# eitan3/xna-ray-trace

Hardware: AMD Instinct MI355X
Metric: Mrays/sec (primary+shadow), 1920×1080; 1/2/4/8-GPU scaling vs HBM roofline (higher is better)
Workload: dtype f32

## Files before the change

### include/xrt.h

```cpp
#ifndef XRT_H
#define XRT_H

#include <stdint.h>

#ifdef __cplusplus
extern "C" {
#endif

#define XRT_VERSION 203

#define XRT_OK              0
#define XRT_E_INVALID_ARG  -1
#define XRT_E_BUSY         -2
#define XRT_E_NO_DEVICE    -3
#define XRT_E_OOM          -4
#define XRT_E_HIP          -5
#define XRT_E_RCCL         -6
#define XRT_E_INTERNAL     -7
#define XRT_E_UNSUPPORTED  -8
#define XRT_E_NOT_BUILT    -9

#define XRT_FILTER_POINT     0
#define XRT_FILTER_BILINEAR  1
#define XRT_ADDRESS_CLAMP    0
// ... 139 lines not shown
                               void *stream);

int xrt_mesh_intersect(xrt_scene *scene, int32_t mesh_id, const xrt_ray *rays, int64_t n,
                       xrt_hit *hits_out);

int xrt_render(xrt_scene *scene, const xrt_camera *camera, const xrt_light *lights, int32_t n_lights,
               const xrt_render_opts *opts, uint32_t *rgba_out, float *rgb_f32_out,
               xrt_stats *stats_out );

int xrt_render_begin(xrt_scene *scene, const xrt_camera *camera, const xrt_light *lights, int32_t n_lights,
                     const xrt_render_opts *opts, uint32_t *rgba_out, int32_t *ticket_out);
int xrt_render_end(xrt_scene *scene, int32_t ticket, xrt_stats *stats_out);

int xrt_host_register(void *host_ptr, uint64_t bytes);
int xrt_host_unregister(void *host_ptr);

int xrt_render_device(xrt_scene *scene, const xrt_camera *camera, const xrt_light *lights,
                      int32_t n_lights, const xrt_render_opts *opts, void *d_rgba_out,
                      void *stream, xrt_stats *stats_out );

int xrt_render_device_begin(xrt_scene *scene, const xrt_camera *camera, const xrt_light *lights,
                            int32_t n_lights, const xrt_render_opts *opts, void *d_rgba_out, void *stream,
                            int32_t *ticket_out);
int xrt_render_device_end(xrt_scene *scene, int32_t ticket, xrt_stats *stats_out);

#define XRT_TILE_W 64
#define XRT_TILE_H 8
int xrt_shard_layout(int32_t width, int32_t height, int32_t shard_count, int32_t *tiles_x_out,
                     int32_t *tiles_y_out, int32_t *tiles_per_rank_out);


int xrt_scene_set_tile_table(xrt_scene *scene, int32_t width, int32_t height, int32_t shard_count, int32_t tiles_per_rank,
                             const int32_t *tile_of_slot);

int xrt_scene_tile_costs(xrt_scene *scene, int32_t width, int32_t height, float *cost_out, int32_t reset);

int xrt_balance_tiles(int32_t width, int32_t height, int32_t shard_count, const float *tile_cost, int32_t tiles_per_rank,
                      int32_t *tile_of_slot_out);

int xrt_detile_table_device(int32_t width, int32_t height, int32_t shard_count, int32_t tiles_per_rank, const void *d_tile_of_slot,
                            const void *d_gathered, int64_t rank_stride, void *d_rgba_out, void *stream);

int xrt_detile_device(int32_t width, int32_t height, int32_t shard_count, const void *d_gathered, int64_t rank_stride,
                      void *d_rgba_out, void *stream);

int xrt_rccl_probe(void);

int xrt_split_stats(xrt_scene *scene, uint64_t out[4], int32_t reset);

int xrt_debug_end_counts(xrt_scene *scene, uint64_t out[3]);

int xrt_debug_packet_table(xrt_scene *scene, uint64_t counts[2], uint32_t *entries_out, int64_t entries_cap, int32_t *paths_out, int64_t paths_cap);

float xrt_progress(const xrt_scene *scene);

int xrt_generate_primary_rays(xrt_scene *scene, const xrt_camera *camera, xrt_ray *rays_out );

int xrt_cast_rays(xrt_scene *scene, const xrt_ray *rays, int64_t n, int32_t iteration, float current_ref_index,
                  const xrt_light *lights, int32_t n_lights, const xrt_render_opts *opts,
                  uint32_t *rgba_out, float *rgb_f32_out, xrt_stats *stats_out );

int xrt_cast_rays_device(xrt_scene *scene, const void *d_rays, int64_t n, int32_t iteration, float current_ref_index,
                         const xrt_light *lights, int32_t n_lights, const xrt_render_opts *opts,
                         void *d_rgba_out, void *d_rgb_f32_out, void *stream, xrt_stats *stats_out );

int xrt_shade_hits(xrt_scene *scene, const xrt_ray *rays, const xrt_hit *hits, int64_t n,
                   int32_t iteration, float current_ref_index,
                   const xrt_light *lights, int32_t n_lights, const xrt_render_opts *opts,
                   uint32_t *rgba_out, float *rgb_f32_out , xrt_stats *stats_out );

int xrt_shade_hits_device(xrt_scene *scene, const void *d_rays, const void *d_hits, int64_t n,
                          int32_t iteration, float current_ref_index,
                          const xrt_light *lights, int32_t n_lights, const xrt_render_opts *opts,
                          void *d_rgba_out, void *d_rgb_f32_out , void *stream,
                          xrt_stats *stats_out );

int xrt_light_hits(xrt_scene *scene, const xrt_hit *hits, int64_t n,
                   const xrt_light *lights, int32_t n_lights,
                   float *light_f32_out , float *amount_out ,
                   xrt_stats *stats_out );

int xrt_light_hits_device(xrt_scene *scene, const void *d_hits, int64_t n,
                          const xrt_light *lights, int32_t n_lights,
                          void *d_light_f32_out, void *d_amount_out , void *stream,
                          xrt_stats *stats_out );

#define XRT_SURF_HIT          1
#define XRT_SURF_TRANSPARENT  2
#define XRT_SURF_INTERPOLATED 4
#define XRT_SURF_TEXTURED     8

typedef struct xrt_surface {
    float   normal[3];
    float   reflectiveness;
    float   color[3];
    float   alpha;
    float   uv[2];
    float   refraction_index;
    float   next_ref_index;
    int32_t flags;
    int32_t reserved[3];
} xrt_surface;

int xrt_surface_hits(xrt_scene *scene, const xrt_ray *rays , const xrt_hit *hits, int64_t n,
                     float current_ref_index, const xrt_render_opts *opts,
                     xrt_surface *surface_out , xrt_ray *reflect_out ,
// ... 85 lines not shown
```

### xna-ray-trace_amd/_abi.py

```python
import ctypes as C
import os

_HERE = os.path.dirname(os.path.abspath(__file__))
import re


def _lib_name():
    v = os.environ.get("XRT_LIB_VARIANT", "libxrt.so")
    if not re.fullmatch(r"libxrt(_\w+)?\.so", v):
        raise ImportError("XRT_LIB_VARIANT=%r: expected libxrt[_name].so (a file inside %s)" % (v, os.path.join(_HERE, "csrc")))
    return v


LIB_PATH = os.path.join(_HERE, "csrc", _lib_name())

XRT_OK = 0
XRT_E_INVALID_ARG = -1
XRT_E_BUSY = -2
XRT_E_NO_DEVICE = -3
XRT_E_OOM = -4
XRT_E_HIP = -5
XRT_E_RCCL = -6
XRT_E_INTERNAL = -7
XRT_E_UNSUPPORTED = -8
# ... 64 lines not shown
    _fields_ = [("position", C.c_float * 3), ("color", C.c_uint32)]


class xrt_surface(C.Structure):
    _fields_ = [("normal", C.c_float * 3), ("reflectiveness", C.c_float), ("color", C.c_float * 3), ("alpha", C.c_float),
                ("uv", C.c_float * 2), ("refraction_index", C.c_float), ("next_ref_index", C.c_float), ("flags", C.c_int32),
                ("reserved", C.c_int32 * 3)]


SURF_HIT, SURF_TRANSPARENT, SURF_INTERPOLATED, SURF_TEXTURED = 1, 2, 4, 8
SURFACE_DTYPE = [("normal", "<f4", 3), ("reflectiveness", "<f4"), ("color", "<f4", 3), ("alpha", "<f4"), ("uv", "<f4", 2),
                 ("refraction_index", "<f4"), ("next_ref_index", "<f4"), ("flags", "<i4"), ("reserved", "<i4", 3)]
assert C.sizeof(xrt_surface) == 64
assert C.sizeof(xrt_path_vertex) == 16
assert C.sizeof(xrt_ray) == 32 and C.sizeof(xrt_hit) == 48 and C.sizeof(xrt_render_opts) == 48
XRT_VERSION = 203

_P = C.POINTER
_F = _P(C.c_float)
SYMBOLS = {
    "xrt_version": (C.c_int, []),
    "xrt_last_error": (C.c_char_p, []),
    "xrt_device_count": (C.c_int, [_P(C.c_int)]),
    "xrt_scene_create": (C.c_int, [C.c_int, _P(C.c_void_p)]),
    "xrt_scene_destroy": (C.c_int, [C.c_void_p]),
    "xrt_scene_add_mesh": (C.c_int, [C.c_void_p, _F, _F, _F, _F, _F, C.c_int32, _P(xrt_material), _F, _P(C.c_int32)]),
    "xrt_scene_add_object": (C.c_int, [C.c_void_p, _P(C.c_int32), C.c_int32, _F, _F, _F, _F, _P(C.c_int32)]),
    "xrt_scene_build": (C.c_int, [C.c_void_p, C.c_int32, C.c_int32]),
    "xrt_scene_save": (C.c_int, [C.c_void_p, C.c_char_p]),
    "xrt_scene_load": (C.c_int, [C.c_int, C.c_char_p, _P(C.c_void_p)]),
    "xrt_scene_get_tree": (C.c_int, [C.c_void_p, C.c_int32, _P(xrt_node_info), _P(C.c_int64), _P(C.c_int32), _P(C.c_int64)]),
    "xrt_scene_intersect": (C.c_int, [C.c_void_p, _P(xrt_ray), _P(C.c_int32), C.c_int64, _P(xrt_hit), _P(xrt_stats)]),
    "xrt_scene_intersect_device": (C.c_int, [C.c_void_p, C.c_void_p, C.c_int64, C.c_void_p, C.c_void_p]),
    "xrt_mesh_intersect": (C.c_int, [C.c_void_p, C.c_int32, _P(xrt_ray), C.c_int64, _P(xrt_hit)]),
    "xrt_render": (C.c_int, [C.c_void_p, _P(xrt_camera), _P(xrt_light), C.c_int32, _P(xrt_render_opts), _P(C.c_uint32), _F, _P(xrt_stats)]),
    "xrt_render_begin": (C.c_int, [C.c_void_p, _P(xrt_camera), _P(xrt_light), C.c_int32, _P(xrt_render_opts), _P(C.c_uint32), _P(C.c_int32)]),
    "xrt_render_end": (C.c_int, [C.c_void_p, C.c_int32, _P(xrt_stats)]),
    "xrt_host_register": (C.c_int, [C.c_void_p, C.c_uint64]),
    "xrt_host_unregister": (C.c_int, [C.c_void_p]),
    "xrt_render_device": (C.c_int, [C.c_void_p, _P(xrt_camera), _P(xrt_light), C.c_int32, _P(xrt_render_opts), C.c_void_p, C.c_void_p, _P(xrt_stats)]),
    "xrt_render_device_begin": (C.c_int, [C.c_void_p, _P(xrt_camera), _P(xrt_light), C.c_int32, _P(xrt_render_opts), C.c_void_p, C.c_void_p, _P(C.c_int32)]),
    "xrt_render_device_end": (C.c_int, [C.c_void_p, C.c_int32, _P(xrt_stats)]),
    "xrt_shard_layout": (C.c_int, [C.c_int32, C.c_int32, C.c_int32, _P(C.c_int32), _P(C.c_int32), _P(C.c_int32)]),
    "xrt_detile_device": (C.c_int, [C.c_int32, C.c_int32, C.c_int32, C.c_void_p, C.c_int64, C.c_void_p, C.c_void_p]),
    "xrt_scene_set_tile_table": (C.c_int, [C.c_void_p, C.c_int32, C.c_int32, C.c_int32, C.c_int32, _P(C.c_int32)]),
    "xrt_scene_tile_costs": (C.c_int, [C.c_void_p, C.c_int32, C.c_int32, _F, C.c_int32]),
    "xrt_balance_tiles": (C.c_int, [C.c_int32, C.c_int32, C.c_int32, _F, C.c_int32, _P(C.c_int32)]),
    "xrt_detile_table_device": (C.c_int, [C.c_int32, C.c_int32, C.c_int32, C.c_int32, C.c_void_p, C.c_void_p, C.c_int64, C.c_void_p, C.c_void_p]),
    "xrt_progress": (C.c_float, [C.c_void_p]),
    "xrt_rccl_probe": (C.c_int, []),
    "xrt_split_stats": (C.c_int, [C.c_void_p, _P(C.c_uint64), C.c_int32]),
    "xrt_debug_end_counts": (C.c_int, [C.c_void_p, _P(C.c_uint64)]),
    "xrt_debug_packet_table": (C.c_int, [C.c_void_p, _P(C.c_uint64), _P(C.c_uint32), C.c_int64, _P(C.c_int32), C.c_int64]),
    "xrt_generate_primary_rays": (C.c_int, [C.c_void_p, _P(xrt_camera), _P(xrt_ray)]),
    "xrt_cast_rays": (C.c_int, [C.c_void_p, _P(xrt_ray), C.c_int64, C.c_int32, C.c_float, _P(xrt_light), C.c_int32, _P(xrt_render_opts),
                                _P(C.c_uint32), _F, _P(xrt_stats)]),
    "xrt_cast_rays_device": (C.c_int, [C.c_void_p, C.c_void_p, C.c_int64, C.c_int32, C.c_float, _P(xrt_light), C.c_int32, _P(xrt_render_opts),
                                       C.c_void_p, C.c_void_p, C.c_void_p, _P(xrt_stats)]),
    "xrt_shade_hits": (C.c_int, [C.c_void_p, _P(xrt_ray), _P(xrt_hit), C.c_int64, C.c_int32, C.c_float, _P(xrt_light), C.c_int32,
                                 _P(xrt_render_opts), _P(C.c_uint32), _F, _P(xrt_stats)]),
    "xrt_shade_hits_device": (C.c_int, [C.c_void_p, C.c_void_p, C.c_void_p, C.c_int64, C.c_int32, C.c_float, _P(xrt_light), C.c_int32,
                                        _P(xrt_render_opts), C.c_void_p, C.c_void_p, C.c_void_p, _P(xrt_stats)]),
    "xrt_light_hits": (C.c_int, [C.c_void_p, _P(xrt_hit), C.c_int64, _P(xrt_light), C.c_int32, _F, _F, _P(xrt_stats)]),
    "xrt_light_hits_device": (C.c_int, [C.c_void_p, C.c_void_p, C.c_int64, _P(xrt_light), C.c_int32, C.c_void_p, C.c_void_p, C.c_void_p, _P(xrt_stats)]),
    "xrt_surface_hits": (C.c_int, [C.c_void_p, _P(xrt_ray), _P(xrt_hit), C.c_int64, C.c_float, _P(xrt_render_opts), _P(xrt_surface), _P(xrt_ray), _P(xrt_ray),
                                   _P(xrt_stats)]),
    "xrt_surface_hits_device": (C.c_int, [C.c_void_p, C.c_void_p, C.c_void_p, C.c_int64, C.c_float, _P(xrt_render_opts), C.c_void_p, C.c_void_p, C.c_void_p,
                                          C.c_void_p, _P(xrt_stats)]),
    "xrt_compose_hits": (C.c_int, [C.c_void_p, _P(xrt_surface), _F, _P(C.c_uint32), _P(C.c_uint32), C.c_int64, _P(C.c_uint32), _F, _P(xrt_stats)]),
    "xrt_compose_hits_device": (C.c_int, [C.c_void_p, C.c_void_p, C.c_void_p, C.c_void_p, C.c_void_p, C.c_int64, C.c_void_p, C.c_void_p, C.c_void_p,
                                          _P(xrt_stats)]),
    "xrt_fold_samples": (C.c_int, [C.c_void_p, _P(C.c_uint32), C.c_int64, C.c_int32, _P(C.c_uint32), _F, _P(xrt_stats)]),
    "xrt_fold_samples_device": (C.c_int, [C.c_void_p, C.c_void_p, C.c_int64, C.c_int32, C.c_void_p, C.c_void_p, C.c_void_p, _P(xrt_stats)]),
    "xrt_cast_rays_paths": (C.c_int, [C.c_void_p, _P(xrt_ray), C.c_int64, C.c_int32, C.c_float, _P(xrt_light), C.c_int32, _P(xrt_render_opts),
                                      _P(C.c_uint32), _F, _P(xrt_ray), _P(C.c_int64), _P(xrt_path_vertex), C.c_int64, _P(C.c_int64), _P(xrt_stats)]),
    "xrt_cast_rays_paths_device": (C.c_int, [C.c_void_p, C.c_void_p, C.c_int64, C.c_int32, C.c_float, _P(xrt_light), C.c_int32, _P(xrt_render_opts),
                                             C.c_void_p, C.c_void_p, C.c_void_p, C.c_void_p, C.c_void_p, C.c_int64, C.c_void_p, _P(C.c_int64), _P(xrt_stats)]),
    "xrt_scene_set_poses": (C.c_int, [C.c_void_p, _P(C.c_int32), C.c_int32, _F, _F, _F]),
    "xrt_scene_set_poses_device": (C.c_int, [C.c_void_p, C.c_void_p, C.c_int32, C.c_void_p, C.c_void_p, C.c_void_p, C.c_void_p]),
    "xrt_scene_build_tree": (C.c_int, [C.c_void_p, C.c_int32]),
    "xrt_scene_set_materials": (C.c_int, [C.c_void_p, _P(C.c_int32), C.c_int32, _P(xrt_material)]),
    "xrt_scene_set_bodies": (C.c_int, [C.c_void_p, C.c_int32, _P(C.c_int32), _P(C.c_int32), _P(C.c_float), _P(C.c_float), _P(C.c_float),
                                       _P(C.c_float), C.c_int32, _P(C.c_int32)]),
    "xrt_scene_set_triangle_shading": (C.c_int, [C.c_void_p, C.c_int32, _P(C.c_int32), C.c_int32, C.c_int32, _F, _F, _F]),
    "xrt_scene_set_triangle_shading_device": (C.c_int, [C.c_void_p, C.c_int32, C.c_void_p, C.c_int32, C.c_int32, C.c_void_p, C.c_void_p, C.c_void_p,
                                                        C.c_void_p]),
    "xrt_render_pixels": (C.c_int, [C.c_void_p, _P(xrt_camera), _P(xrt_light), C.c_int32, _P(xrt_render_opts), _F, C.c_int64, _P(C.c_uint32), _F,
                                    _P(xrt_stats)]),
    "xrt_render_pixels_device": (C.c_int, [C.c_void_p, _P(xrt_camera), _P(xrt_light), C.c_int32, _P(xrt_render_opts), C.c_void_p, C.c_int64,
                                           C.c_void_p, C.c_void_p, C.c_void_p, _P(xrt_stats)]),
    "xrt_trace_pixels": (C.c_int, [C.c_void_p, _P(xrt_camera), _P(xrt_render_opts), _F, C.c_int64, _P(xrt_ray), _P(xrt_hit), _P(xrt_stats)]),
    "xrt_trace_pixels_device": (C.c_int, [C.c_void_p, _P(xrt_camera), _P(xrt_render_opts), C.c_void_p, C.c_int64, C.c_void_p, C.c_void_p, C.c_void_p,
                                          _P(xrt_stats)]),
}

_lib = None


class XrtError(RuntimeError):
    def __init__(self, code, msg):
        super().__init__("libxrt error %d: %s" % (code, msg))
        self.code = code


def lib():
    global _lib
# ... 28 lines not shown
```

### xna-ray-trace_amd/api.py

```python
import ctypes as C
import threading
import numpy as np

from . import _abi as abi
from . import xna

f32 = np.float32


def _fp(a):
    return a.ctypes.data_as(C.POINTER(C.c_float))


def _material_property(name, convert, texels=False):
    attr = "_" + name

    def get(self):
        return getattr(self, attr)

    def set_(self, value):
        setattr(self, attr, convert(value))
        self._serial = getattr(self, "_serial", 0) + 1
        if texels:
            self._tex_serial = getattr(self, "_tex_serial", 0) + 1
# ... 440 lines not shown
        some = next((t for t in (ids, normals, uv, color) if t is not None), None)
        s = stream if stream is not None else torch.cuda.current_stream(some.device if some is not None else None)
        ptr = lambda t: C.c_void_p(t.data_ptr()) if t is not None else None
        abi.check(abi.lib().xrt_scene_set_triangle_shading_device(self.handle, int(mesh_id), ptr(ids), first, n, ptr(normals), ptr(uv), ptr(color),
                                                                  C.c_void_p(s.cuda_stream)))
        if 0 <= mesh_id < len(self.meshes):
            hids = np.arange(first, first + n, dtype=np.int64) if ids is None else ids.detach().cpu().numpy()
            keep = (hids >= 0) & (hids < self.meshes[mesh_id].data.ntri)
            host = lambda t, shape: None if t is None else t.detach().cpu().numpy().reshape(shape)[keep]
            self._mirror_triangle_shading(int(mesh_id), hids[keep], 0, int(keep.sum()), host(normals, (n, 3, 3)), host(uv, (n, 3, 2)),
                                          host(color, (n, 4)))

    def Save(self, path):
        self._push_materials()
        abi.check(abi.lib().xrt_scene_save(self.handle, str(path).encode()))

    @classmethod
    def Load(cls, path, device=0):
        sm = cls(device)
        sm._scene = _Scene.__new__(_Scene)
        sm._scene.handle = C.c_void_p()
        abi.check(abi.lib().xrt_scene_load(int(device), str(path).encode(), C.byref(sm._scene.handle)))
        abi.check(abi.lib().xrt_scene_build(sm._scene.handle, sm.meshItemTreshold, sm.itemTreshold))
        return sm

    @property
    def handle(self):
        if self._scene is None:
            raise RuntimeError("scene not built")
        return self._scene.handle

    def mesh_id(self, mesh):
        return self._mesh_ids[id(mesh)]

    def SplitStats(self, reset=True):
        out = (C.c_uint64 * 4)()
        abi.check(abi.lib().xrt_split_stats(self.handle, out, 1 if reset else 0))
        return tuple(int(x) for x in out)

    def EndCounts(self):
        out = (C.c_uint64 * 3)()
        abi.check(abi.lib().xrt_debug_end_counts(self.handle, out))
        return tuple(int(x) for x in out)

    def PacketTable(self):
        counts = (C.c_uint64 * 2)()
        abi.check(abi.lib().xrt_debug_packet_table(self.handle, counts, None, 0, None, 0))
        entries = np.zeros((int(counts[0]), 2), dtype=np.uint32)
        paths = np.zeros(int(counts[1]), dtype=np.int32)
        abi.check(abi.lib().xrt_debug_packet_table(self.handle, counts, entries.ctypes.data_as(C.POINTER(C.c_uint32)), entries.shape[0],
                                                   paths.ctypes.data_as(C.POINTER(C.c_int32)), paths.shape[0]))
        return entries, paths

    def IntersectBatch(self, rays, stats=False):
        rays = np.ascontiguousarray(rays, dtype=RAY_DTYPE)
        hits = np.zeros(rays.shape[0], dtype=HIT_DTYPE)
        st = abi.xrt_stats()
        self._push_poses()
        self._push_materials()
        abi.check(abi.lib().xrt_scene_intersect(self.handle, rays.ctypes.data_as(C.POINTER(abi.xrt_ray)), None, rays.shape[0],
                                                hits.ctypes.data_as(C.POINTER(abi.xrt_hit)), C.byref(st) if stats else None))
        return (hits, st.as_dict()) if stats else hits

    def GetRayIntersection(self, ray, ignoreTriangle=None, ignoreObject=None):
        im, it = (-1, -1) if ignoreTriangle is None else (self.mesh_id(ignoreTriangle[0]), int(ignoreTriangle[1]))
        h = self.IntersectBatch(rays_array([ray[0]], [ray[1]], im, it))[0]
        if not h["hit"]:
            return False, None
        return True, dict(mesh=self.meshes[h["mesh"]], triangle=int(h["tri"]), u=h["u"], v=h["v"], d=h["d"],
                          worldPosition=h["w"].copy(), object=int(h["object"]), leaf=int(h["leaf"]))

    def tree(self, mesh=None):
        return _get_tree(self._scene, -1 if mesh is None else self.mesh_id(mesh))


class Camera:

    def __init__(self, position, target, up, fieldOfView, aspectRatio, nearClippingPlane, farClippingPlane):
        self.Position, self.Target, self.Up = position, target, up
        self.FieldOfView, self.AspectRatio = fieldOfView, aspectRatio
        self.NearClippingPlane, self.FarClippingPlane = nearClippingPlane, farClippingPlane

    @property
    def View(self):
        return xna.as_array(xna.create_look_at(self.Position, self.Target, self.Up))

    @property
    def Projection(self):
        return xna.as_array(xna.create_perspective_fov(self.FieldOfView, self.AspectRatio, self.NearClippingPlane, self.FarClippingPlane))


class SpotLight:
    IsPositionable = True

    def __init__(self):
        self.Position = (0.0, 0.0, 0.0)
        self.Direction = (0.0, -1.0, 0.0)
        self.Color = (1.0, 1.0, 1.0)
        self.DecayExponent = 1.3
        self.Intensity = 1.0
        self.SpotAngle = 0.0

    def _to_abi(self):
        l = abi.xrt_light()
        l.kind = abi.LIGHT_SPOT
        l.position[:] = self.Position
# ... 520 lines not shown
```

### xna-ray-trace_amd/csrc/frame_plan.h

```cpp
#pragma once
#include "../../include/xrt.h"
#include "kernels.h"

struct xrt_scene;
namespace xrt { struct PixelGenArgs; }

struct BatchSrc {
    const xrt_ray *rays = nullptr;
    long long n = 0;
    float refIndex = 1.0f;
    struct Paths {
        xrt_path_vertex *vertices = nullptr;
        long long capacity = 0;
        long long *vertexStart = nullptr;
        xrt_ray *raysBack = nullptr;
    };
    const Paths *paths = nullptr;
    const xrt_hit *hits = nullptr;
    bool coherent = false;
    int samples = 1;
    const xrt::PixelGenArgs *gen = nullptr;
};

constexpr int ADAPTIVE_LEVEL_WORDS = 16;

struct FramePlan {
    xrt::RayGenParams g{};
    int R = 0, nL = 0;
    int addressMode = 0, filtering = 0;
    bool tabled = false;
    long long totalTiles = 0, myTiles = 0, totalPixels = 0;
    long long framePaths = 0;
    long long partStart = 0, firstPaths = 0;
    long long hintPaths = -1;
    unsigned long long validPixels = 0;
    size_t nodes = 0;
    long long chunkPaths = 0;
    int P = 0;
    size_t rayCap = 0, liveCap = 0, lvlStride = 0, shadowCap = 0;
    int cntStride = 0, qStride = 0;
    bool lvlVerified = false;
    bool heap = false;
    bool adaptive = false;
    int quality = 0;
    bool batch = false, capturePaths = false;
    bool givenHits = false;
    bool collect = false;
    bool fast = false;
    bool heapFast = false;
    bool adaptiveFast = false;
    bool ae = false;
    bool finishA = false;
    bool endEarly = false;
    bool skipTiles = false;
    unsigned long long endSkipped = 0;
    bool fuseResolve = false;
    bool wantF32 = false;
    bool wantFeedback = false;
    bool listLong = false;
    bool hinted = false;
    bool tileCosts = false;
    bool useStamps = false;
    int pkMask = 0;
    size_t pkEntries = 0;
    int shadeBlock = 1024;
    bool ownStream = false;
    int cntBase = 0, levelCap = 0;
};

int plan_frame(const xrt_scene &s, int matVersion, const xrt_camera *cam, const xrt_light *lights, int nLights, const xrt_render_opts *opts, bool wantsF32,
               bool hasStream, int part, int nParts, bool heapFastAllowed, const BatchSrc *batch, FramePlan &plan);

int scene_packet_mask(const xrt_scene &s, int samples);
bool scene_answers_at_emission(const xrt_scene &s);
```

### xna-ray-trace_amd/csrc/kernels.h

```cpp
#pragma once
#include <hip/hip_runtime.h>

#include "../../include/xrt.h"
#include "traverse.h"

namespace xrt {

struct ShadeView {
    const f4 *shade;
    const MaterialRec *materials;
    const uint32_t *texels;
    const MeshRec *meshes;
    const LightRec *lights;
    int nLights;
    int addressMode, filtering;
};

struct HeavyArgs {
    int *list = nullptr;
    int *count = nullptr;
    float path = 0.0f;
    const unsigned *costMap = nullptr;
    unsigned epoch = 0;
    int costThreshold = 0;
// ... 17 lines not shown
    int batchMax = 64;
    int heavyShift = 3;
    int batchMin = 64;
    int spreadMin = 4;
    unsigned long long *stamps = nullptr;
    const xrt_ray *rays2 = nullptr;
    xrt_hit *hits2 = nullptr;
    const int *nDev2 = nullptr;
    int nMul2 = 0, nCap2 = 0;
    int *flags = nullptr, *flags2 = nullptr;
    int missRecords = 0;
    const int *scatter = nullptr, *scatter2 = nullptr;
};

constexpr int STAMP_HEADER = 2, STAMP_SLOTS = 8192, STAMP_STRIDE = STAMP_HEADER + STAMP_SLOTS;

struct alignas(16) SlotRec { float wx, wy, wz; int path; float nx, ny, nz, refl; };
struct PacketArgs {
    const xrt_ray *rays = nullptr;
    xrt_hit *hits = nullptr;
    const int *index = nullptr;
    const int *nDev = nullptr;
    int nMul = 1, n = 0, nCap = 0;
    unsigned *queue = nullptr;
    int mode = MODE_SINGLE, meshId = 0;
    int unmark = 0;
    int staticDiv = 4;
    int grabMax = 2;
    int *flags = nullptr;
    int splitLong = 0, splitBudgetLong = 0;
    int cullMin = 4;
    unsigned long long *stamps = nullptr;
    const xrt_ray *rays2 = nullptr;
    xrt_hit *hits2 = nullptr;
    int *flags2 = nullptr;
    const int *nDev2 = nullptr;
    int nMul2 = 0, nCap2 = 0;
    const int *scatter = nullptr, *scatter2 = nullptr;
    unsigned *tileCost = nullptr;
    int tileShift = 9, nL1 = 1, nL2 = 1, tileBase = 0;
    const int *pathOf1 = nullptr;
    const SlotRec *slotOf1 = nullptr;
    const SlotRec *slotOf2 = nullptr;
    unsigned *splitCtl = nullptr;
    unsigned *splitItems = nullptr;
    unsigned *splitRecs = nullptr;
    int splitNI = 0, splitNR = 0;
    unsigned splitSerial = 0;
    int splitBudget = 0, splitBudgetItem = 0;
    unsigned *splitCost = nullptr;
    const uint2 *pkTable = nullptr;
    const unsigned *pkCount = nullptr;
    int pkCap = 0;
};
struct QuadTable {
    uint2 *table = nullptr;
    unsigned *count = nullptr, *clear = nullptr;
    int cap = 0;
};
constexpr int QUAD_HEAD_WORDS = 128;
constexpr int PACKET_QUEUE_HEADS = 8, PACKET_HEAD_STRIDE = 64;
constexpr int PACKET_SPLIT_WORDS = 320;
constexpr int PACKET_QUEUE_WORDS = PACKET_QUEUE_HEADS * PACKET_HEAD_STRIDE + PACKET_SPLIT_WORDS;
constexpr int SPLIT_HEAD_WORDS = 32, SPLIT_PART_WORDS = 7 * 64, SPLIT_ITEM_WORDS = SPLIT_HEAD_WORDS + 64 + SPLIT_PART_WORDS, SPLIT_REC_HEAD = 64, SPLIT_REC_WORDS = SPLIT_REC_HEAD + SPLIT_PART_WORDS;
constexpr int SPLIT_REC_ITEMS = 32;
int  packet_split_stats(unsigned long long out[4], bool reset);
bool packet_supported(int mode, int meshDepth, int sceneDepth);
int  packet_blocks_per_cu(int mode);
void launch_packet(const SceneView &S, const PacketArgs &A, int gridBlocks, hipStream_t st, hipEvent_t e0 = nullptr, hipEvent_t e1 = nullptr);

enum { C_RAYS = 0, C_HITS, C_SCENE_NODES, C_INSTANCES, C_MESH_AABB, C_MESH_QUERIES, C_NODES, C_REFS, C_TRIS, C_MESH_AWAY, C_COUNT };

constexpr int FLAG_MISS = 0, FLAG_HIT = 1, FLAG_TRANSPARENT = 2;


enum { END_LISTED = 0, END_BY_RAYGEN, END_BY_SHADE, END_WORDS };
struct EndArgs {
    int on = 0;
    uint32_t *sampleColor = nullptr;
    int *list = nullptr, *cnt = nullptr;
    int listCap = 0;
    int skipTiles = 0;
};

struct ShadeArgs {
    int level, doA, doB;
    int maxReflections, P, heap;
    int *overflow;
    const xrt_ray *rays; const xrt_hit *hits;
    const int *nDev; int nHost, cap;
    const int *index, *rayPath, *rayNode; const float *rayRef;
    SlotRec *slotOut; int *slotNodeOut; int *scnt; int shadowCap; xrt_ray *shadowRays;
    xrt_ray *nextRays; int *nextPath, *nextNode; float *nextRef; int *nextCnt; int nextCap;
    const SlotRec *slotPrev; const int *slotNodePrev; const int *scntPrev; const xrt_hit *shadowHits;
    f4 *lvlA, *lvlB; float *lvlAlpha;
    LvlMap lvl;
    HeavyArgs heavy;
    unsigned *costOut = nullptr;
    unsigned epoch = 0;
    const int *hitFlags = nullptr, *shadowFlags = nullptr;
    int ae = 0;
    int *shadowCnt = nullptr, *shadowOut = nullptr, *shadowFlagsOut = nullptr;
    int finish = 0;
    int *finishCnt = nullptr;
    EndArgs end;
};

void launch_intersect(const SceneView &S, const IntersectArgs &A, int stackNeeded, int gridBlocks, hipStream_t st, hipEvent_t e0 = nullptr,
                      hipEvent_t e1 = nullptr);
int  intersect_blocks_per_cu(int stackNeeded, int mode);
void launch_count(const SceneView &S, const IntersectArgs &A, unsigned long long *counters, hipStream_t st);
void launch_raygen(const RayGenParams &g, const SceneView &S, xrt_ray *rays, f4 *lvlB0, int *index, int *count, int P, long long pathBase,
// ... 93 lines not shown
```

### xna-ray-trace_amd/csrc/kernels.hip

```cpp
#include "kernels.h"
#include "device_util.h"
#include "pose.h"
#include "shade_math.h"

#include <hip/hip_ext.h>

namespace xrt {

struct LdsStack {
    unsigned *base;
    __device__ __forceinline__ unsigned get(int i) const { return base[i * 64]; }
    __device__ __forceinline__ void set(int i, unsigned v) { base[i * 64] = v; }
};

__device__ __forceinline__ int wave_scan_max(int v) {
    v = max(v, __builtin_amdgcn_update_dpp(0, v, 0x111, 0xf, 0xf, false));
    v = max(v, __builtin_amdgcn_update_dpp(0, v, 0x112, 0xf, 0xf, false));
    v = max(v, __builtin_amdgcn_update_dpp(0, v, 0x114, 0xf, 0xf, false));
    v = max(v, __builtin_amdgcn_update_dpp(0, v, 0x118, 0xf, 0xf, false));
    v = max(v, __builtin_amdgcn_update_dpp(0, v, 0x142, 0xa, 0xf, false));
    v = max(v, __builtin_amdgcn_update_dpp(0, v, 0x143, 0xc, 0xf, false));
    return v;
}

constexpr int APPEND_BLOCK = 1024;
__device__ __forceinline__ int block_append(int *counter, bool flag, int *ldsCounts ) {
    const unsigned long long m = __ballot(flag);
    const int wave = (int)(threadIdx.x >> 6), nw = (int)(blockDim.x >> 6), lane = lane_id();
    if (lane == 0) ldsCounts[wave] = (int)__popcll(m);
    __syncthreads();
    if (wave == 0) {
        const int c = lane < nw ? ldsCounts[lane] : 0;
        const int incl = wave_scan_add(c);
        const int total = __builtin_amdgcn_readlane(incl, 63);
        int base = 0;
        if (lane == 0 && total) base = atomicAdd(counter, total);
        base = __builtin_amdgcn_readfirstlane(base);
        if (lane < nw) ldsCounts[lane] = base + incl - c;
    }
    __syncthreads();
    const int slot = ldsCounts[wave] + lanes_below(m);
    __syncthreads();
    return slot;
}

__device__ __forceinline__ void block_count(int *counter, int n, int *ldsCounts ) {
    const int wave = (int)(threadIdx.x >> 6), nw = (int)(blockDim.x >> 6), lane = lane_id();
    const int mine = __builtin_amdgcn_readlane(wave_scan_add(n), 63);
    __syncthreads();
    if (lane == 0) ldsCounts[wave] = mine;
    __syncthreads();
    if (wave == 0) {
        const int total = __builtin_amdgcn_readlane(wave_scan_add(lane < nw ? ldsCounts[lane] : 0), 63);
        if (lane == 0 && total) atomicAdd(counter, total);
    }
// ... 483 lines not shown
            const int q = grp * span + r * APPEND_BLOCK + (int)threadIdx.x;
            const int p = path_of(q);
            bool live = false, heavy = false, record = true;
            keepO[r] = mk(0, 0, 0); keepD[r] = mk(0, 0, 0);
            if (q < walk && p < P) {
                long long gp = pathBase + p;
                const int sshift = g.samples == 16 ? 4 : (g.samples == 4 ? 2 : 0);
                int s = (int)(gp & (long long)(g.samples - 1));
                int x = 0, y = 0;
                const bool listed = g.quadLevel > 0;
                if (!listed && !path_pixel(g, gp >> sshift, x, y)) {
                    if (!index) store_ray(rays + p, mk(0, 0, 0), mk(0, 0, 0), DEAD_RAY, -1);
                    record = g.cullSkipsRecord == 0;
                } else if (index && !listed && (x < g.cullX0 || x > g.cullX1 || y < g.cullY0 || y > g.cullY1)) {
                    record = g.cullSkipsRecord == 0;
                } else {
                    float sx = (float)x, sy = (float)y;
                    if (g.quadLevel >= 0) {
                        if (listed) { sx = g.quadCx[gp >> 2]; sy = g.quadCy[gp >> 2]; }
                        const float quarter = g.quadSize * 0.25f;
                        sx = (s & 1) ? sx + quarter : sx - quarter;
                        sy = (s & 2) ? sy + quarter : sy - quarter;
                    } else if (g.samples == 16) {
                        int q = s >> 2, rr = s & 3;
                        sx = (sx + ((q & 1) ? 0.25f : -0.25f)) + ((rr & 1) ? 0.125f : -0.125f);
                        sy = (sy + ((q & 2) ? 0.25f : -0.25f)) + ((rr & 2) ? 0.125f : -0.125f);
                    }
                    v3 nearP = unproject(g, sx, sy, 0.0f);
                    v3 farP = unproject(g, sx, sy, 1.0f);
                    v3 dir = normalize(sub(farP, nearP));
                    if (index) {
                        RayPre w = make_ray(nearP, dir);
                        float key;
                        live = slab(w, rlo.x, rlo.y, rlo.z, rhi.x, rhi.y, rhi.z, key);
                    }
                    heavy = live && H.list && long_ray(S, H, p, nearP, dir);
                    if (!index) store_ray(rays + p, nearP, dir, -1, -1);
                    keepO[r] = nearP; keepD[r] = dir;
                }
                if constexpr (END) { if (!live) { sample_color_out(E.sampleColor, nullptr, p, pack_color(mk(0, 0, 0)), mk(0, 0, 0)); nEnded++; } }
                else if (index && !live && record) lvlB0[lvl_at(g.lvl, p)] = f4{0, 0, 0, i2f(FLAG_MISS)};
            }
            const unsigned long long ml = __ballot(live), mh = __ballot(heavy);
            liveAt[r] = live ? lanes_below(ml) : -1;
            heavyAt[r] = heavy ? lanes_below(mh) : -1;
            if (lane == 0) { ldsLive[r * 16 + wave] = (int)__popcll(ml); ldsHeavy[r * 16 + wave] = (int)__popcll(mh); }
        }
        if (!index) continue;
        __syncthreads();
        int quadLen = 0, quadAt = 0;
        if (wave == 0 && Q.table) reserve_cells_and_entries(ldsLive, count, Q.count, quadLen, quadAt);
        else if (wave < 2 && (wave == 0 || H.list)) reserve_cells(wave == 0 ? ldsLive : ldsHeavy, wave == 0 ? count : H.count);
        __syncthreads();
        if (quadLen > 0 && quadAt < Q.cap) Q.table[quadAt] = make_uint2((unsigned)ldsLive[lane], (unsigned)quadLen);
#pragma unroll
        for (int r = 0; r < RG_ROUNDS; r++) {
            const int p = path_of(grp * span + r * APPEND_BLOCK + (int)threadIdx.x);
            if (liveAt[r] >= 0) {
                const int slot = ldsLive[r * 16 + wave] + liveAt[r];
                if (slot < liveCap) {
                    index[slot] = p;
                    store_ray(rays + slot, keepO[r], keepD[r], -1, heavyAt[r] >= 0 ? (-1 ^ HEAVY_BIT) : -1);
                    if (heavyAt[r] >= 0) H.list[ldsHeavy[r * 16 + wave] + heavyAt[r]] = slot;
                }
            }
        }
        __syncthreads();
    }
    if constexpr (END) block_count(E.cnt + END_BY_RAYGEN, nEnded, ldsLive);
}
__global__ __launch_bounds__(APPEND_BLOCK) void k_ingest(RayGenParams g, SceneView S, xrt_ray *rays, f4 *lvlB0, int *index, int *count, int P,
                                                         long long pathBase, HeavyArgs H, int liveCap) {
    __shared__ int ldsLive[RG_ROUNDS * 16], ldsHeavy[RG_ROUNDS * 16];
    const f4 rlo = S.snodes[0], rhi = S.snodes[1];
    const int span = RG_ROUNDS * APPEND_BLOCK;
    const int groups = (P + span - 1) / span;
    const int wave = (int)(threadIdx.x >> 6), lane = lane_id();
    for (int grp = (int)blockIdx.x; grp < groups; grp += (int)gridDim.x) {
        int liveAt[RG_ROUNDS], heavyAt[RG_ROUNDS];
        f4 keepA[RG_ROUNDS], keepB[RG_ROUNDS];
#pragma unroll
        for (int r = 0; r < RG_ROUNDS; r++) {
            const int p = grp * span + r * APPEND_BLOCK + (int)threadIdx.x;
            bool live = false, heavy = false;
            keepA[r] = f4{0, 0, 0, 0}; keepB[r] = f4{0, 0, 0, 0};
            if (p < P) {
                const f4 *src = g.batch + 2 * (size_t)(pathBase + p);
                const f4 a = src[0], b = src[1];
                const v3 o = mk(a.x, a.y, a.z), d = mk(a.w, b.x, b.y);
                int im = f2i(b.z), it = f2i(b.w);
                if (it < 0 || im < 0 || im >= S.nMeshes || it >= S.meshes[im].ntri) { im = -1; it = -1; }
                RayPre w = make_ray(o, d);
                float key;
                live = slab(w, rlo.x, rlo.y, rlo.z, rhi.x, rhi.y, rhi.z, key);
                heavy = live && H.list && long_ray(S, H, p, o, d);
                keepA[r] = a;
                keepB[r] = f4{b.x, b.y, i2f(im), i2f(heavy ? (it ^ HEAVY_BIT) : it)};
                if (!live) lvlB0[p] = f4{0, 0, 0, i2f(FLAG_MISS)};
            }
            const unsigned long long ml = __ballot(live), mh = __ballot(heavy);
            liveAt[r] = live ? lanes_below(ml) : -1;
            heavyAt[r] = heavy ? lanes_below(mh) : -1;
            if (lane == 0) { ldsLive[r * 16 + wave] = (int)__popcll(ml); ldsHeavy[r * 16 + wave] = (int)__popcll(mh); }
        }
        __syncthreads();
        if (wave < 2 && (wave == 0 || H.list)) reserve_cells(wave == 0 ? ldsLive : ldsHeavy, wave == 0 ? count : H.count);
        __syncthreads();
// ... 679 lines not shown
```

### xna-ray-trace_amd/csrc/packet.hip

```cpp
#include "device_util.h"
#include "kernels.h"

#include <hip/hip_ext.h>

namespace xrt {

constexpr int PK_LEVELS = 24;
constexpr int PK_FRAME_WORDS = 4;
constexpr int PK_SPLIT_AT = PK_LEVELS * (PK_FRAME_WORDS + 16);
constexpr int PK_STACK_WORDS = PK_SPLIT_AT + 8 + 24;
static_assert(PK_STACK_WORDS == 512, "a wave's stack is 2 KB");
constexpr int PK_SLEVELS = 12;
constexpr int PK_SFRAME_WORDS = 4;
constexpr int PK_QUEUES = 8;
static_assert(PK_QUEUES >= 1 && PK_QUEUES <= PACKET_QUEUE_HEADS, "the host zeroes PACKET_QUEUE_WORDS heads per packet launch");
#ifndef PK_SINGLE_WAVES
#define PK_SINGLE_WAVES 6
#endif
constexpr int PK_SGPRS = PK_SINGLE_WAVES >= 7 ? 96 : 112;

#if defined(XRT_PK_COUNTERS) && !defined(XRT_PK_TICKS)
#define XRT_PK_TICKS
#endif
#ifdef XRT_PK_TICKS
__device__ unsigned long long g_pkWorst[16];
__device__ unsigned g_pkDump[2 * 65536];
__device__ unsigned long long g_pkTicks[32];
#endif
#ifdef XRT_PK_COUNTERS
__device__ unsigned long long g_pkCounters[16];
__device__ unsigned g_pkCur[8 * 65536];
#define PKC(i) (pkc[i]++)
#else
#define PKC(i) ((void)0)
#endif

__device__ unsigned long long g_splitStats[4];
struct alignas(4) TriWords { float w[16]; };
__device__ __forceinline__ int rfl(int v) { return __builtin_amdgcn_readfirstlane(v); }
__device__ __forceinline__ unsigned ld_ag(const unsigned *p) { return __hip_atomic_load(p, __ATOMIC_RELAXED, __HIP_MEMORY_SCOPE_AGENT); }
__device__ __forceinline__ void st_ag(unsigned *p, unsigned v) { __hip_atomic_store(p, v, __ATOMIC_RELAXED, __HIP_MEMORY_SCOPE_AGENT); }
__device__ __forceinline__ void stores_done() { __builtin_amdgcn_fence(__ATOMIC_RELEASE, "workgroup"); asm volatile("s_waitcnt vmcnt(0)" ::: "memory"); }
__device__ __forceinline__ void loads_after() { __builtin_amdgcn_fence(__ATOMIC_ACQUIRE, "workgroup"); }
__device__ __forceinline__ unsigned xcc_id() { return (unsigned)__builtin_amdgcn_s_getreg(20 | (0 << 6) | ((4 - 1) << 11)) & 7u; }
__device__ __forceinline__ float rflf(float v) { return i2f(__builtin_amdgcn_readfirstlane(f2i(v))); }

struct PkUniform {
    int blk, p, dm0;
    unsigned long long lanes;
};
struct alignas(16) PkBlockWords { float w[PBLOCK_WORDS]; };
struct alignas(16) Frame4 { unsigned a, b, c, d; };
__device__ __forceinline__ int pk_hit8_fast(const RayPre &r, const PkBlockWords &B) {
    const float tx0 = (B.w[8] - r.o.x) * r.inv.x, tx1 = (B.w[9] - r.o.x) * r.inv.x, tx2 = (B.w[10] - r.o.x) * r.inv.x;
// ... 72 lines not shown
    L.mfound = 1;
    L.mKey = better ? L.leafKey : L.mKey; L.mDist = better ? t : L.mDist; L.mU = better ? u : L.mU; L.mV = better ? v : L.mV;
    L.mRef = better ? r : L.mRef; L.mLeaf = better ? L.leafNode : L.mLeaf;
}

template <class KeyFn>
__device__ __forceinline__ void pk_scan_leaf(const float *__restrict__ refT, int r0, int r1, Lane &L, const SceneView &S, bool keyed, KeyFn entry_key) {
    const char *pt = reinterpret_cast<const char *>(refT) + (size_t)r0 * TRI_REC_BYTES;
    auto test = [&](const TriWords &q, int r) {
        float u, v, t;
        PkTriMid m;
        if (pk_tri_pre(q, L, m)) {
            if (pk_tri_hit(q, L, m, u, v, t)) {
                if (!keyed) L.leafKey = entry_key();
                pk_candidate(L, S, r, u, v, t);
            }
        }
    };
    TriWords qA = *reinterpret_cast<const TriWords *>(pt);
    int r = r0;
    for (;;) {
        const TriWords qB = *reinterpret_cast<const TriWords *>(pt + TRI_REC_BYTES);
        test(qA, r);
        if (r + 1 >= r1) break;
        qA = *reinterpret_cast<const TriWords *>(pt + 2 * TRI_REC_BYTES);
        test(qB, r + 1);
        r += 2; pt += 2 * TRI_REC_BYTES;
        if (r >= r1) break;
    }
}

constexpr unsigned PK_KERNARG_SCENE = 8 * 8, PK_KERNARG_ARGS = PK_KERNARG_SCENE + (unsigned)sizeof(SceneView);
static_assert(sizeof(SceneView) % 8 == 0 && alignof(PacketArgs) == 8, "kernel-argument offsets of k_packet");
typedef const __attribute__((address_space(4))) PacketArgs *PkArgsK;
typedef const __attribute__((address_space(4))) SceneView *PkSceneK;
struct PkKernarg {
    unsigned long long base;
    __device__ __forceinline__ PkKernarg() : base((unsigned long long)__builtin_amdgcn_kernarg_segment_ptr()) {}
    __device__ __forceinline__ void fresh() {
        unsigned lo = (unsigned)__builtin_amdgcn_readfirstlane((int)(unsigned)base), hi = (unsigned)__builtin_amdgcn_readfirstlane((int)(unsigned)(base >> 32));
        asm volatile("" : "+s"(lo), "+s"(hi));
        base = (unsigned long long)lo | ((unsigned long long)hi << 32);
    }
    __device__ __forceinline__ PkArgsK args() const { return (PkArgsK)(base + PK_KERNARG_ARGS); }
    __device__ __forceinline__ PkSceneK scene() const { return (PkSceneK)(base + PK_KERNARG_SCENE); }
    __device__ __forceinline__ SceneView result_view() const {
        const PkSceneK k = scene();
        SceneView v = {};
        v.refG = k->refG; v.refN = k->refN; v.meshes = k->meshes; v.childDfs = k->childDfs; v.objects = k->objects;
        return v;
    }
};

template <bool SPLIT, bool LEAF_RHO>
__device__ __forceinline__ void pk_walk(const float *__restrict__ pblocks, const float *__restrict__ refT, const float *__restrict__ lrec,
                                        const SceneView &S, int cullMin, unsigned *stk, int lane, Lane &L,
                                        const RayCull &RC, bool fastL, int rootBlock, unsigned long long lanes0, bool nodeCull,
                                        bool resume) {
#ifdef XRT_PK_COUNTERS
    unsigned pkc[16] = {0, 0, 0, 0, 0, 0, 0, 0, 0, 0, 0, 0, 0, 0, 0, 0};
    pkc[0] = 1;
    pkc[12] = (unsigned)__popcll(lanes0);
#endif
    PkUniform U;
    U.blk = rootBlock;
    U.lanes = lanes0;
    U.p = 0; U.dm0 = 0;
    unsigned char *const cbOf = reinterpret_cast<unsigned char *>(stk + PK_LEVELS * PK_FRAME_WORDS) + lane;
    int sp = resume ? 1 : 0;
    bool entering = !resume, anyFound = resume && __any(L.mfound != 0);
    PkBlockWords B;
    int cb = 0;
    unsigned *const sst = stk + PK_SPLIT_AT;
    auto spill = [&]() {
        PkKernarg K;
        K.fresh();
        const PkArgsK a = K.args();
        unsigned *const ctl = a->splitCtl, *const itemsB = a->splitItems, *const recsB = a->splitRecs;
        const int NR = a->splitNR;
        const unsigned serial = a->splitSerial, xcc = xcc_id(), NIx = (unsigned)a->splitNI / 8u;
        const unsigned takerBudget = (unsigned)a->splitBudgetItem, takerEvery = (unsigned)rfl((int)sst[7]);
        int rec = rfl((int)sst[0]);
        for (int lvl = 0; lvl < sp; lvl++) {
            const Frame4 f = *reinterpret_cast<const Frame4 *>(stk + lvl * PK_FRAME_WORDS);
            const unsigned p = (unsigned)rfl((int)f.b);
            if (p == 0u) continue;
            if (rec < 0) {
                unsigned r = 0u;
                if (lane == 0) r = atomicAdd(ctl + 256, 1u);
                rec = rfl((int)r);
                if (rec >= NR) { rec = -1; break; }
                if (lane == 0) {
                    unsigned *const R0 = recsB + (size_t)rec * SPLIT_REC_WORDS;
                    (void)atomicExch(R0, 1u); (void)atomicExch(R0 + 1, 0u);
                    sst[0] = (unsigned)rec;
                    atomicAdd(&g_splitStats[2], 1ull);
                }
            }
            unsigned *const R = recsB + (size_t)rec * SPLIT_REC_WORDS;
            unsigned j = 0u, idx = 0u;
            if (lane == 0) j = atomicAdd(R + 1, 1u);
            j = (unsigned)rfl((int)j);
            if (j >= (unsigned)SPLIT_REC_ITEMS) break;
            if (lane == 0) idx = atomicAdd(ctl + 32u * xcc, 1u);
            idx = (unsigned)rfl((int)idx);
            if (idx >= NIx) { if (lane == 0) st_ag(R + 32 + j, 0xffffffffu); break; }
            idx += xcc * NIx;
// ... 35 lines not shown
                    }
                }
            }
            B = *reinterpret_cast<const PkBlockWords *>(pblocks + (size_t)U.blk * PBLOCK_WORDS);
            cb = 0;
            if (in) cb = fastL ? pk_hit8_fast(L.r, B) : pk_hit8_slow(L.r, B);
            cb &= 0xff & ~((f2i(B.w[2]) >> 8) & 0xff);
            U.dm0 = __builtin_amdgcn_readlane(L.dmask, (int)__builtin_ctzll(U.lanes));
            const int a4 = U.dm0 & 4, a2 = U.dm0 & 2, a1 = U.dm0 & 1;
            int q = cb;
            q = ((q << a4) | (q >> a4)) & 0xff;
            q = ((q & 0x33) << a2) | ((q & 0xcc) >> a2);
            q = ((q & 0x55) << a1) | ((q & 0xaa) >> a1);
            U.p = wave_or(q);
            entering = false;
        }
        if (U.p == 0) {
            if (sp == 0) break;
            sp--;
            PKC(10);
            const Frame4 f = *reinterpret_cast<const Frame4 *>(stk + sp * PK_FRAME_WORDS);
            U.blk = rfl((int)f.a); U.p = rfl((int)f.b);
            U.lanes = (unsigned long long)(unsigned)rfl((int)f.c) | ((unsigned long long)(unsigned)rfl((int)f.d) << 32);
            U.dm0 = __builtin_amdgcn_readlane(L.dmask, (int)__builtin_ctzll(U.lanes));
            B = *reinterpret_cast<const PkBlockWords *>(pblocks + (size_t)U.blk * PBLOCK_WORDS);
            cb = (int)cbOf[sp * 64];
            continue;
        }
        const int c = (int)__builtin_ctz((unsigned)U.p) ^ U.dm0;
        U.p &= U.p - 1;
        PKC(2);
        const bool inC = in && ((cb >> c) & 1);
        const int d0 = f2i(B.w[0]), d1 = f2i(B.w[1]), d2 = f2i(B.w[2]), d3 = f2i(B.w[3]);
        auto entry_key = [&]() {
            v3 cmin, cmax;
            pk_child_box(B, c, cmin, cmax);
            float k = 0.0f;
            if (fastL) (void)slab_fast(L.r, L.dmask, cmin, cmax, k);
            else (void)slab(L.r, cmin.x, cmin.y, cmin.z, cmax.x, cmax.y, cmax.z, k);
            return k;
        };
        const bool keyed = anyFound;
        float key = 0.0f;
        if (keyed && inC) key = entry_key();
#ifdef XRT_PK_COUNTERS
        if (keyed) pkc[11]++;
        pkc[13] += (unsigned)__popcll(__ballot(inC));
#endif
        const int node = U.blk * 8 + c;
        if (!((d2 >> c) & 1)) {
            PKC(3);
            const f4 *const nr = reinterpret_cast<const f4 *>(lrec + (size_t)node * LREC_WORDS);
            const f4 nlo = nr[0], nhi = nr[1];
            bool go = inC & !all_back_facing(nlo, nhi, L.r.d);
            if (keyed) go = go & !((L.mfound != 0) & (key > L.mKey));
            if (!__any(go)) continue;
            PKC(4);
            const unsigned long long offLo = (unsigned long long)(unsigned)f2i(B.w[4]) | ((unsigned long long)(unsigned)f2i(B.w[5]) << 32);
            const unsigned long long offHi = (unsigned long long)(unsigned)f2i(B.w[6]) | ((unsigned long long)(unsigned)f2i(B.w[7]) << 32);
            const int r0 = d1 + child_ref_offset(offLo, offHi, c);
            const int r1 = d1 + ((c == 7) ? d3 : child_ref_offset(offLo, offHi, c + 1));
            const bool big = r1 - r0 >= LEAF_RUN_MIN;
            float rho = 0.0f;
            bool usable = false;
            if constexpr (LEAF_RHO) {
                if (big || r1 - r0 >= cullMin) {
                    usable = leaf_margin(L.r, RC, nr[2], nr[3], nr[4], nr[5], rho);
                    if (r1 - r0 >= cullMin) {
                        go = go && !(usable && grown_box_missed(L.r, nr[2], nr[3], rho));
                        if (!__any(go)) continue;
                    }
                }
            } else if (r1 - r0 >= cullMin) {
                go = go && !leaf_certainly_missed_fused(L.r, RC, nr[2], nr[3], nr[4], nr[5]);
                if (!__any(go)) continue;
            }
            PKC(5);
            int nRuns = 1, rb = -1;
            if (big) { rb = f2i(lrec[(size_t)node * LREC_WORDS + 24]); if (rb >= 0) nRuns = (r1 - r0 + LEAF_RUN - 1) / LEAF_RUN; }
            const bool cheap = LEAF_RHO && !__any(go && !usable);
            for (int jr = 0; jr < nRuns; jr++) {
                int ra = r0, rz = r1;
                bool goR = go;
                if (rb >= 0) {
                    ra = r0 + LEAF_RUN * jr; rz = min(ra + LEAF_RUN, r1);
                    const f4 *tb = reinterpret_cast<const f4 *>(lrec + (size_t)rb + (size_t)jr * RUN_WORDS);
                    PKC(6);
                    if (cheap) goR = go && !grown_box_missed(L.r, tb[0], tb[1], rho);
                    else if constexpr (LEAF_RHO) goR = go && !leaf_certainly_missed(L.r, RC, tb[0], tb[1], tb[2], tb[3]);
                    else goR = go && !leaf_certainly_missed_fused(L.r, RC, tb[0], tb[1], tb[2], tb[3]);
                    if (!__any(goR)) continue;
                }
                PKC(7);
#ifdef XRT_PK_COUNTERS
                pkc[8] += (unsigned)(rz - ra);
                pkc[14] += (unsigned)(rz - ra) * (unsigned)__popcll(__ballot(goR));
#endif
                if (goR) {
                    L.leafKey = key; L.leafNode = node;
                    const char *pt = reinterpret_cast<const char *>(refT) + (size_t)ra * TRI_REC_BYTES;
                    auto test = [&](const TriWords &q, int r) {
                        float u, v, t;
                        PkTriMid m;
                        if (pk_tri_pre(q, L, m)) {
                            if (pk_tri_hit(q, L, m, u, v, t)) {
                                if (!keyed) L.leafKey = entry_key();
                                pk_candidate(L, S, r, u, v, t);
                            }
                        }
                    };
                    TriWords qA = *reinterpret_cast<const TriWords *>(pt);
                    int r = ra;
                    for (;;) {
                        const TriWords qB = *reinterpret_cast<const TriWords *>(pt + TRI_REC_BYTES);
                        test(qA, r);
                        if (r + 1 >= rz) break;
                        qA = *reinterpret_cast<const TriWords *>(pt + 2 * TRI_REC_BYTES);
                        test(qB, r + 1);
                        r += 2; pt += 2 * TRI_REC_BYTES;
                        if (r >= rz) break;
                    }
                }
            }
            if (!keyed) anyFound = __any(L.mfound != 0);
            continue;
        }
        bool go = inC;
        if (keyed && ((d2 >> (16 + c)) & 1)) go = go & !((L.mfound != 0) & (key > L.mKey));
        if (nodeCull && ((d2 >> (24 + c)) & 1)) {
            const f4 *const nr = reinterpret_cast<const f4 *>(lrec + (size_t)node * LREC_WORDS);
            go = go && !all_back_facing(nr[0], nr[1], L.r.d);
            PKC(9);
        }
        const unsigned long long LL = __ballot(go);
        if (LL == 0ull) continue;
        if (sp >= PK_LEVELS - 1) continue;
        if (U.p != 0) {
            cbOf[sp * 64] = (unsigned char)cb;
            if (lane == 0) *reinterpret_cast<Frame4 *>(stk + sp * PK_FRAME_WORDS) = Frame4{(unsigned)U.blk, (unsigned)U.p, (unsigned)U.lanes, (unsigned)(U.lanes >> 32)};
            __builtin_amdgcn_fence(__ATOMIC_RELEASE, "wavefront");
            __builtin_amdgcn_wave_barrier();
            __builtin_amdgcn_fence(__ATOMIC_ACQUIRE, "wavefront");
            sp++;
        }
        U.blk = d0 + __builtin_popcount((unsigned)(d2 & 0xff) & ((1u << c) - 1u));
        U.lanes = LL;
        entering = true;
    }
#ifdef XRT_PK_COUNTERS
    if (lane == 0) for (int i = 0; i < 16; i++) if (pkc[i]) atomicAdd(&g_pkCounters[i], (unsigned long long)pkc[i]);
    if (lane == 0) {
        unsigned *cur = g_pkCur + 8 * ((blockIdx.x * 4 + (threadIdx.x >> 6)) & 65535);
        cur[0] += pkc[0]; cur[1] += pkc[1]; cur[2] += pkc[2]; cur[3] += pkc[8]; cur[4] += pkc[6];
    }
#endif
}

constexpr int PK_PARK_WORDS = 19;
struct PkScene {
    LdsRay w;
    LdsField<float> sKey;
    LdsField<int> sfound;
    LdsField<float> sbKey, sbD, sbU, sbV;
    LdsField<int> sbRef, sbLeaf, sbObj, sbMesh;
    int obj;
    __device__ __forceinline__ explicit PkScene(unsigned *b)
        : w{b}, sKey{b + 9 * 64}, sfound{b + 10 * 64}, sbKey{b + 11 * 64}, sbD{b + 12 * 64}, sbU{b + 13 * 64}, sbV{b + 14 * 64},
          sbRef{b + 15 * 64}, sbLeaf{b + 16 * 64}, sbObj{b + 17 * 64}, sbMesh{b + 18 * 64}, obj(-1) {}
};
template <int M> __device__ __forceinline__ unsigned *scene_park() {
    if constexpr (M == MODE_SCENE) { __shared__ unsigned mem[4 * PK_PARK_WORDS * 64]; return mem; }
    else return nullptr;
}
template <int M> __device__ __forceinline__ unsigned *scene_frames() {
    if constexpr (M == MODE_SCENE) { __shared__ unsigned mem[4 * PK_SLEVELS * PK_SFRAME_WORDS]; return mem; }
    else return nullptr;
}

#ifndef PK_SCENE_WAVES
#define PK_SCENE_WAVES 5
#endif
template <int M, bool SP>
__global__ __launch_bounds__(256, (M == MODE_SCENE) ? PK_SCENE_WAVES : (PK_SINGLE_WAVES >= 7 ? 7 : (SP ? 6 : 1))) __attribute__((amdgpu_num_sgpr(PK_SGPRS))) void k_packet(const float *__restrict__ pblocks, const float *__restrict__ refT,
                                                const float *__restrict__ lrec, const MeshRec *__restrict__ meshes,
                                                const f4 *__restrict__ snodes, const f4 *__restrict__ scull, const ObjRec *__restrict__ objects,
                                                const int *__restrict__ objMesh, SceneView S, PacketArgs A) {
    __shared__ unsigned frames[4 * PK_STACK_WORDS];
    unsigned *const sframesAll = scene_frames<M>();
    unsigned *const parkAll = scene_park<M>();
    stamp_begin(A.stamps);
    PkKernarg KA;
    const int lane = lane_id(), wave = (int)(threadIdx.x >> 6);
    unsigned *const stk = &frames[wave * PK_STACK_WORDS];
    int n = A.nDev ? (*A.nDev) * A.nMul : A.n;
    if (A.nCap > 0 && n > A.nCap) n = A.nCap;
    int n2 = A.nDev2 ? (*A.nDev2) * A.nMul2 : 0;
    if (n2 > A.nCap2) n2 = A.nCap2;
    int nPkT = (n + 63) >> 6;
    if (A.pkTable) { const int t = (int)*A.pkCount; nPkT = t > A.pkCap ? A.pkCap : t; }
    const int nPk1 = nPkT, nPk = nPk1 + ((n2 + 63) >> 6);
    const int nWaves = (int)gridDim.x * 4, waveId = (int)blockIdx.x * 4 + wave;
    int staticPer = A.staticDiv > 0 ? nPk / (nWaves * A.staticDiv) : 0;
    if (staticPer == 0) staticPer = 1;
    const int qBase = min(nWaves * staticPer, nPk);
    const int dynTotal = nPk - qBase;
    unsigned dead = 0u;
    for (int h = 0; h < PK_QUEUES; h++) if (dynTotal - h <= 0) dead |= 1u << h;
    int cur = waveId % PK_QUEUES, seen = 0, curR = cur;
    int sNext = 0, dNext = 0, dEnd = 0;
    constexpr bool splitOn = SP && M != MODE_SCENE;
    unsigned *const sst = stk + PK_SPLIT_AT;
    if (splitOn && lane == 0) sst[2] = 0u;
    bool mainDone = false;
    for (;;) {
        int pk = -1, item = -1;
        bool contended = false;
        if (splitOn) {
            KA.fresh();
            const unsigned xcc = xcc_id(), NIx = (unsigned)KA.args()->splitNI / 8u;
            unsigned *const ctl = KA.args()->splitCtl + 32u * xcc;
            unsigned long long th = 0ull;
            if (lane == 0) th = __hip_atomic_load(reinterpret_cast<unsigned long long *>(ctl), __ATOMIC_RELAXED, __HIP_MEMORY_SCOPE_AGENT);
            const unsigned t = (unsigned)rfl((int)(unsigned)th), h = (unsigned)rfl((int)(unsigned)(th >> 32));
            if (h < (t < NIx ? t : NIx)) {
                unsigned old = 0u;
                if (lane == 0) old = atomicCAS(ctl + 1, h, h + 1u);
                if ((unsigned)rfl((int)old) == h) item = (int)(xcc * NIx + h);
                else contended = true;
            }
        }
        if (item < 0) {
            if (mainDone) {
                if (!contended) break;
                __builtin_amdgcn_s_sleep(8);
                continue;
            }
// ... 65 lines not shown
#else
        const bool costed = KA.args()->tileCost != nullptr || (splitOn && KA.args()->splitCost != nullptr);
#endif
        const unsigned long long tPacket = costed ? wall_clock64() : 0ull;
        const bool seg2 = pk >= nPk1;
        int w = (seg2 ? pk - nPk1 : pk) * 64 + lane;
        bool valid = w < (seg2 ? n2 : n);
        if (!seg2) {
            const uint2 *const tab = KA.args()->pkTable;
            if (tab) {
                const uint2 e = tab[pk];
                w = rfl((int)e.x) + lane;
                valid = lane < rfl((int)e.y) && w < n;
            }
        }
        const xrt_ray *const raysS = seg2 ? KA.args()->rays2 : KA.args()->rays;
        Lane L;
        L.state = ST_FINISH; L.mfound = 0; L.cost = 0; L.rayIndex = 0; L.mesh = 0; L.weird = 0; L.dmask = 0; L.ignoreId = -1; L.mask = 0;
        L.r = make_ray(mk(0, 0, 0), mk(1, 1, 1));
        int idx = 0;
        v3 o = mk(0, 0, 0), d = mk(0, 0, 0);
        int im = DEAD_RAY, it = -1;
        if (valid) {
            const int *const indexL = KA.args()->index;
            idx = (indexL && !seg2) ? indexL[w] : w;
            load_ray(raysS + idx, o, d, im, it);
            if (KA.args()->unmark && heavy_marked(it)) it ^= HEAVY_BIT;
        }
        if constexpr (M != MODE_SCENE) {
            SceneLane C;
            C.sfound = 0; C.obj = 0;
            if (valid && im != DEAD_RAY) lane_begin(L, C, S, o, d, im, it, idx, M, A.meshId, false);
            const RayCull RC = make_ray_cull(L.r.o, L.r.d);
            const int mesh = (M == MODE_MESH) ? A.meshId : 0;
            const MeshRec &mr = meshes[mesh];
            const bool fastL = L.r.par == 0 && L.weird == 0;
            const bool nodeCull = S.nodeCull == 2 || (S.nodeCull == 1 && __any(valid && L.ignoreId >= 0));
            const bool meshAway = nodeCull && mesh_faces_away(mr, L.r.d);
            unsigned long long lanes0 = mr.rootBlock < 0 ? 0ull : __ballot(valid && L.state == ST_NODE && L.mask != 0 && !meshAway);
            if (splitOn) {
                if (item >= 0) {
                    const unsigned *const P = itemW + SPLIT_HEAD_WORDS + 64 + lane;
                    L.mfound = (int)ld_ag(P); L.mKey = i2f((int)ld_ag(P + 64)); L.mDist = i2f((int)ld_ag(P + 128)); L.mU = i2f((int)ld_ag(P + 192)); L.mV = i2f((int)ld_ag(P + 256));
                    L.mRef = (int)ld_ag(P + 320); L.mLeaf = (int)ld_ag(P + 384);
                    reinterpret_cast<unsigned char *>(stk + PK_LEVELS * PK_FRAME_WORDS)[lane] = (unsigned char)ld_ag(itemW + SPLIT_HEAD_WORDS + lane);
                    const unsigned hw = lane < 4 ? ld_ag(itemW + 3 + lane) : 0u;
                    if (lane < 4) stk[lane] = hw;
                    lanes0 = (unsigned long long)(unsigned)__builtin_amdgcn_readlane((int)hw, 2) | ((unsigned long long)(unsigned)__builtin_amdgcn_readlane((int)hw, 3) << 32);
                    __builtin_amdgcn_fence(__ATOMIC_RELEASE, "wavefront");
                    __builtin_amdgcn_wave_barrier();
                    __builtin_amdgcn_fence(__ATOMIC_ACQUIRE, "wavefront");
                }
            }
            pk_walk<splitOn, true>(pblocks, refT, lrec, S, A.cullMin, stk, lane, L, RC, fastL, mr.rootBlock, lanes0, nodeCull, splitOn && item >= 0);
            L.mesh = mesh;
            KA.fresh();
            bool mine = true;
            if (splitOn) {
                const int rec = rfl((int)sst[0]);
                if (rec >= 0) {
                    const int itemA = rfl((int)sst[1]);
                    unsigned *const R = KA.args()->splitRecs + (size_t)rec * SPLIT_REC_WORDS;
                    unsigned *const P = (itemA >= 0 ? KA.args()->splitItems + (size_t)itemA * SPLIT_ITEM_WORDS + SPLIT_HEAD_WORDS + 64 : R + SPLIT_REC_HEAD) + lane;
                    st_ag(P, (unsigned)L.mfound); st_ag(P + 64, (unsigned)f2i(L.mKey)); st_ag(P + 128, (unsigned)f2i(L.mDist)); st_ag(P + 192, (unsigned)f2i(L.mU)); st_ag(P + 256, (unsigned)f2i(L.mV));
                    st_ag(P + 320, (unsigned)L.mRef); st_ag(P + 384, (unsigned)L.mLeaf);
                    stores_done();
                    unsigned left = 0u;
                    if (lane == 0) left = atomicSub(R, 1u);
                    mine = rfl((int)left) == 1;
                    if (mine) {
                        loads_after();
                        if (itemA >= 0 && lane == 0) atomicAdd(&g_splitStats[3], 1ull);
                        const SceneView Sr = KA.result_view();
                        int nIt = rfl((int)__hip_atomic_load(R + 1, __ATOMIC_RELAXED, __HIP_MEMORY_SCOPE_AGENT));
                        if (nIt > SPLIT_REC_ITEMS) nIt = SPLIT_REC_ITEMS;
                        for (int j = -1; j < nIt; j++) {
                            const unsigned *Q = R + SPLIT_REC_HEAD + lane;
                            if (j >= 0) {
                                const unsigned ix = (unsigned)rfl((int)ld_ag(R + 32 + j));
                                if (ix == 0xffffffffu) continue;
                                Q = KA.args()->splitItems + (size_t)ix * SPLIT_ITEM_WORDS + SPLIT_HEAD_WORDS + 64 + lane;
                            }
                            const int qf = (int)ld_ag(Q), qRef = (int)ld_ag(Q + 320), qLeaf = (int)ld_ag(Q + 384);
                            const float qKey = i2f((int)ld_ag(Q + 64)), qD = i2f((int)ld_ag(Q + 128)), qU = i2f((int)ld_ag(Q + 192)), qV = i2f((int)ld_ag(Q + 256));
                            if (qf != 0) {
                                bool better = (L.mfound == 0) | (qKey < L.mKey) | ((qKey == L.mKey) & (qD < L.mDist));
                                if ((L.mfound != 0) & (qKey == L.mKey) & (qD == L.mDist))
                                    better = qLeaf != L.mLeaf ? node_dfs(Sr, qLeaf) < node_dfs(Sr, L.mLeaf) : f2i(Sr.refN[qRef].w) < f2i(Sr.refN[L.mRef].w);
                                if (better) { L.mfound = 1; L.mKey = qKey; L.mDist = qD; L.mU = qU; L.mV = qV; L.mRef = qRef; L.mLeaf = qLeaf; }
                            }
                        }
                    }
                }
            }
            if (valid && mine) {
                const SceneView Sr = KA.result_view();
                const HitOut h = lane_result(L, C, Sr, M);
                xrt_hit *const hitsS = seg2 ? KA.args()->hits2 : KA.args()->hits;
                int *const flagsS = seg2 ? KA.args()->flags2 : KA.args()->flags;
                const int *const scat = seg2 ? KA.args()->scatter2 : KA.args()->scatter;
                const int at = scat ? scat[idx] : idx;
                if (flagsS) flagsS[at] = h.hit;
                if (!flagsS || h.hit) store_hit(hitsS + at, h);
            }
        } else {
            PkScene C(parkAll + wave * PK_PARK_WORDS * 64 + lane);
            unsigned *const sfr = sframesAll + wave * PK_SLEVELS * PK_SFRAME_WORDS;
// ... 52 lines not shown
                    if (go) {
                        const RayPre wr = C.w;
                        const bool weird = L.weird != 0;
                        for (int j = 0; j < nb; j++) {
                            const f4 c0 = rec[4 * j], c1 = rec[4 * j + 1], c2 = rec[4 * j + 2];
                            const bool p = (f2i(c2.y) == 0) | weird | precull_box(wr, c0, c1, c2.x);
                            pass |= (p ? 1u : 0u) << j;
                        }
                    }
                    unsigned any = (unsigned)wave_or((int)pass);
                    while (any != 0u) {
                        const int j = (int)__builtin_ctz(any);
                        any &= any - 1u;
                        const bool inB = ((pass >> j) & 1u) != 0u;
                        const f4 h2 = rec[4 * j + 2], h3 = rec[4 * j + 3];
                        const int o = rfl(f2i(h2.z)), m0 = rfl(f2i(h2.w)), m1 = m0 + rfl(f2i(h3.x));
                        if (inB) {
                            const f4 *const oq = reinterpret_cast<const f4 *>(objects + o);
                            const f4 q0 = oq[0], q1 = oq[1], q2 = oq[2], q3 = oq[3];
                            const float iw[16] = {q0.x, q0.y, q0.z, q0.w, q1.x, q1.y, q1.z, q1.w, q2.x, q2.y, q2.z, q2.w, q3.x, q3.y, q3.z, q3.w};
                            const RayPre wr = C.w;
                            const v3 rayDirPosition = add(wr.o, wr.d);
                            const v3 v1 = transform(wr.o, iw);
                            const v3 v2 = transform(rayDirPosition, iw);
                            const v3 dir = normalize(sub(v2, v1));
                            L.r = make_ray(v1, dir);
                            L.dmask = dir_mask(dir);
                            if (!(is_finite(v1.x) && is_finite(v1.y) && is_finite(v1.z) && is_finite(dir.x) && is_finite(dir.y) && is_finite(dir.z))) L.weird = 1;
                        }
                        const RayCull RC = make_ray_cull(L.r.o, L.r.d);
                        const bool fastL = L.r.par == 0 && L.weird == 0;
                        for (int mi = m0; mi < m1; mi++) {
                            const int m = rfl(objMesh[mi]);
                            const MeshRec &mr = meshes[m];
                            float k;
                            const bool inM = inB && slab(L.r, mr.bmin[0], mr.bmin[1], mr.bmin[2], mr.bmax[0], mr.bmax[1], mr.bmax[2], k);
                            if (!__any(inM)) continue;
                            float rkey = 0.0f;
                            const bool inRoot = inM && slab(L.r, mr.rmin[0], mr.rmin[1], mr.rmin[2], mr.rmax[0], mr.rmax[1], mr.rmax[2], rkey);
                            L.mfound = 0;
                            const int rootBlock = rfl(mr.rootBlock);
                            if (rootBlock < 0) {
                                const int r0 = rfl(mr.rootRef), rc = rfl(mr.rootCount);
                                if (rc > 0 && __any(inRoot)) {
                                    if (inRoot) {
                                        L.leafKey = rkey; L.leafNode = ROOT_NODE;
                                        pk_scan_leaf(refT, r0, r0 + rc, L, S, true, [&]() { return rkey; });
                                    }
                                }
                            } else {
                                const bool meshAway = nodeCull && mesh_faces_away(mr, L.r.d);
                                const unsigned long long lanes0 = __ballot(inRoot && !meshAway);
                                if (lanes0 != 0ull)
                                    pk_walk<false, false>(pblocks, refT, lrec, S, A.cullMin, stk, lane, L, RC, fastL, rootBlock, lanes0, nodeCull, false);
                            }
                            if (L.mfound) {
                                L.mesh = m; C.obj = o;
                                merge_mesh_result(L, C);
                                L.mfound = 0;
                            }
                        }
                    }
                }
            }
            KA.fresh();
            if (valid) {
                L.mfound = 0;
                const SceneView Sr = KA.result_view();
                const HitOut h = lane_result(L, C, Sr, M);
                xrt_hit *const hitsS = seg2 ? KA.args()->hits2 : KA.args()->hits;
                int *const flagsS = seg2 ? KA.args()->flags2 : KA.args()->flags;
                const int *const scat = seg2 ? KA.args()->scatter2 : KA.args()->scatter;
                const int at = scat ? scat[idx] : idx;
                if (flagsS) flagsS[at] = h.hit;
                if (!flagsS || h.hit) store_hit(hitsS + at, h);
            }
        }
        if (costed) {
            const unsigned dt = (unsigned)(wall_clock64() - tPacket);
#ifdef XRT_PK_TICKS
            if (lane == 0) atomicAdd(&g_pkTicks[dt ? 31 - __builtin_clz(dt) : 0], 1ull);
            if (lane == 0 && pk < 65536 && nPk > 4096 && !seg2 && g_pkDump[2 * pk] == 0u) { g_pkDump[2 * pk] = dt; g_pkDump[2 * pk + 1] = stk[PK_SPLIT_AT + 6]; }
            if (lane == 0) stk[PK_SPLIT_AT + 6] = 0u;
            {
                const unsigned long long nv = __popcll(__ballot(valid));
                const unsigned long long nSlow = __popcll(__ballot(valid && (L.r.par != 0 || L.weird != 0)));
                if (lane == 0 && nSlow) { atomicAdd(&g_pkWorst[11], 1ull); atomicAdd(&g_pkWorst[12], (unsigned long long)dt); }
                if (lane == 0) {
#ifdef XRT_PK_COUNTERS
                    unsigned *cur = g_pkCur + 8 * ((blockIdx.x * 4 + (threadIdx.x >> 6)) & 65535);
#else
                    unsigned cur[8] = {0, 0, 0, 0, 0, 0, 0, 0};
#endif
                    if ((unsigned long long)dt > atomicMax(&g_pkWorst[0], (unsigned long long)dt)) {
                        g_pkWorst[1] = (unsigned long long)pk; g_pkWorst[2] = seg2 ? 1ull : 0ull; g_pkWorst[3] = cur[0]; g_pkWorst[4] = cur[1]; g_pkWorst[5] = cur[2];
                        g_pkWorst[6] = cur[3]; g_pkWorst[7] = cur[4]; g_pkWorst[8] = nv; g_pkWorst[9] = (unsigned long long)nPk; g_pkWorst[10] = nSlow;
                    }
                    for (int i = 0; i < 8; i++) cur[i] = 0;
                }
            }
            if (lane == 0 && KA.args()->tileCost) {
#else
            if constexpr (splitOn) {
                if (splitOn && lane == 0 && KA.args()->splitCost && (int)sst[1] < 0) {
                    const unsigned pred = sst[5], mine = sst[6];
                    KA.args()->splitCost[pk] = ((int)sst[0] >= 0 && pred > mine) ? pred : mine;
                }
// ... 82 lines not shown
```

### xna-ray-trace_amd/csrc/scene_state.h

```cpp
#pragma once
#include <condition_variable>
#include <functional>
#include <map>
#include <memory>
#include <thread>

#include "device_res.h"
#include "frame_plan.h"
#include "kernels.h"
#include "paths.h"
#include "rccl_gather.h"
#include "scene_host.h"
#include "settings.h"

struct RankWorker {
    std::thread th;
    std::mutex m;
    std::condition_variable cv;
    std::function<void()> job;
    bool posted = false, finished = false, quit = false;
    explicit RankWorker(int device) {
        th = std::thread([this, device] {
            (void)hipSetDevice(device);
            std::unique_lock<std::mutex> lk(m);
// ... 112 lines not shown
    DevBuf<uint32_t> castRGBA;
    DevBuf<float> castF32;
    DevBuf<xrt_hit> castHits;
    struct LightWork {
        DevBuf<xrt_ray> rays;
        DevBuf<xrt_hit> hits;
        DevBuf<int> flags, scatter, counts;
        DevBuf<unsigned> queue, splitItems, splitRecs;
        DevBuf<LightRec> lights;
        DevBuf<float> lightOut, amountOut;
        Event ev[4];
    } lightWork;
    struct SurfaceWork {
        DevBuf<unsigned long long> count;
        DevBuf<xrt_surface> surfaceOut;
        DevBuf<xrt_ray> reflectOut, refractOut;
        Event ev[2];
    } surfaceWork;
    struct ComposeWork {
        DevBuf<unsigned long long> count;
        DevBuf<xrt_surface> surfaceIn;
        DevBuf<float> lightIn, f32Out;
        DevBuf<uint32_t> reflectIn, refractIn, samplesIn, rgbaOut;
        Event ev[2];
    } composeWork;
    struct TraceWork {
        DevBuf<xrt_ray> rays, countRays, raysOut;
        DevBuf<xrt_hit> hitsOut;
        DevBuf<float> centers;
        DevBuf<int> counts;
        DevBuf<unsigned> queue, splitItems, splitRecs;
        Event ev[4];
    } traceWork;
    DevBuf<f4> pathHit, pathDir;
    DevBuf<int> pathLocal, pathBlockSum;
    DevBuf<long long> pathBlockBase, pathStart;
    DevBuf<xrt_path_vertex> pathVerts;
    DevBuf<xrt_ray> pathBack;
    unsigned pathEpoch = 0;
    Pinned<long long> pathPinned;
    DevBuf<xrt_ray> pixelRays;
    DevBuf<uint32_t> pixelSamples;
    DevBuf<float> pixelCenters;
    DevBuf<unsigned> queues;
    DevBuf<uint32_t> outRGBA;
    DevBuf<float> outF32;
    DevBuf<unsigned long long> counters;
    struct WorkBufs {
        DevBuf<xrt_ray> rays0, rays1, shadowRays;
        DevBuf<xrt_hit> hits, shadowHits;
        DevBuf<int> path0, path1, index0, heavyList, cnts;
        DevBuf<int> composeList;
        DevBuf<unsigned> quadTable;
        int quadWord = 0;
        DevBuf<int> node0, node1, heapFlag;
        DevBuf<float> ref0, ref1, lvlAlpha;
        DevBuf<int> hitFlags0, shadowFlags;
        DevBuf<unsigned> splitCost;
        size_t splitCostStride = 0;
        DevBuf<unsigned> splitItems, splitRecs;
        DevBuf<int> shadowOut;
        DevBuf<int> shadowFlags1;
        DevBuf<unsigned long long> stamps;
        DevBuf<SlotRec> slot0, slot1;
        DevBuf<int> slotNode0, slotNode1;
        DevBuf<f4> lvlA, lvlB;
        DevBuf<uint32_t> sampleColor;
        DevBuf<float> sampleF32;
        DevBuf<LightRec> lights;
        struct Level { DevBuf<uint32_t> color; DevBuf<int> childBase, childMask; DevBuf<float> cx, cy; } levels[8];
        bool levelWordsClean = false;
        bool heapFlagClean = false;
        bool cntsClean = false;
        std::vector<LightRec> lightsOnDevice;
        const void *lightsDevPtr = nullptr;
        Stream stream;
        hipStream_t lastStream = nullptr;
    };
    DevBuf<unsigned> costMap;
    size_t costMapPaths = 0;
    unsigned epoch = 100;
    int costT[66];
    bool deepMeshes = false;
    float heavyPath = 0.0f;
    DevBuf<unsigned long long> waveTimes;
    struct FrameCtx {
        std::vector<Event> events;
        Pinned<int> pinned;
        std::vector<std::pair<size_t, size_t>> pairs;
        size_t ev = 0;
        Event done;
        std::vector<LightRec> hostLights;
        int pose = 0;
        int mat = 0;
        int shade = 0;
        bool pending = false;
        FramePlan plan;
        bool redone = false;
        xrt_camera redoCam; xrt_render_opts redoOpts; std::vector<xrt_light> redoLights;
        uint32_t *redoOut = nullptr; float *redoOutF32 = nullptr; hipStream_t redoSt = nullptr;
        int stampRows = 0;
        Pinned<unsigned long long> stampHost;
        int tallyChunks = 0;
        unsigned long long answered = 0;
        unsigned long long shaded = 0, closestDeep = 0, livePaths = 0, live0 = 0, validPixels = 0;
        unsigned long long hcnt[2 * C_COUNT] = {0};
// ... 46 lines not shown
```

### xna-ray-trace_amd/csrc/settings.h

```cpp
#pragma once

#include <climits>
#include <cstdio>
#include <cstdlib>
#include <optional>
#include <string>
#include <type_traits>

namespace xrt {

constexpr int MAX_CHUNK_PATHS = 1 << 25;
constexpr int HEAP_RAY_CAP = 1 << 22;
constexpr int MAX_STAMP_ROWS = 256;

struct Settings {
    int packetMask = -1;
    int packetMaskHeap = -1;
    int batchMax = 64;
    int batchMin = 64;
    int spreadMin = 4;
    int tune[4] = {0, 16, 48, 32};
    std::optional<int> heavyShift;
    std::optional<int> firstBatch;
    bool packetMerge = true;
    bool answerAtEmission = true;
    bool finishInPartA = true;
    bool endEarly = true;
    int packetCullMin = 4;
    bool packetSplit = false;
    int packetBudgetUs = 350, packetBudgetItemUs = 150, packetSplitItems = 8192;
    int packetLongUs = 0, packetBudgetLongUs = 8;
    int packetGrabMax = 2;
    int packetStaticDiv = 4;
    bool packetQuads = true;
    bool levelMap = true;
    int nodeCull = 1;
    bool noSingle = false;
    int longFracLo = 2, longFracHi = 6;
    std::optional<float> heavy;
    long long heapRayCap = HEAP_RAY_CAP;
    long long shadowBytes = 8LL << 30;
    long long maxChunkPaths = MAX_CHUNK_PATHS;
    long long pixelBytes = 4LL << 30;
    float overlapMinMs = 0.05f;
    std::optional<int> splitMode;
    int splitParts = 2;
    float splitMinMs = 1.0f;
    bool launchEvents = false;
    int maxStampRows = MAX_STAMP_ROWS;
    bool adaptiveFast = true;
    long long adaptiveCap = 0;
    bool heapFast = true;
    bool gridHints = true;
    int shadeBlock = 768;
    bool launchTiming = true;
    std::string waveTimesPath;
    std::string stampDumpPath;
    bool fakeGpus = false;
    bool noRectCull = false, oneStream = false, noFeedback = false;
    std::optional<bool> spatialRuns;
#ifdef XRT_DEV
    std::optional<double> leafCullSafety;
    std::optional<double> cullSafety;
    bool finishCounts = false;
#endif
    std::optional<bool> guard;
};

template <class T>
void env_int(const char *name, T &out, long long lo, long long hi, long long step = 1) {
    const char *e = getenv(name);
    if (!e) return;
    const long long v = std::is_same<T, long long>::value ? atoll(e) : atoi(e);
    if (v >= lo && v <= hi && v % step == 0) out = T(v);
}
template <class T>
void env_flag(const char *name, T &out) { if (const char *e = getenv(name)) out = atoi(e) != 0; }
template <class T>
void env_float(const char *name, T &out) { if (const char *e = getenv(name)) out = (float)atof(e); }
inline void env_str(const char *name, std::string &out) { if (const char *e = getenv(name)) out = e; }
inline bool env_set(const char *name) { return getenv(name) != nullptr; }

inline Settings read_settings() {
    Settings c;
    env_int("XRT_PACKET", c.packetMask, -1, 31);
    env_int("XRT_PACKET_HEAP", c.packetMaskHeap, -1, 31);
    env_int("XRT_BATCH_MAX", c.batchMax, 16, 4096, 16);
    env_int("XRT_BATCH_MIN", c.batchMin, 16, 64, 16);
    env_int("XRT_SPREAD_MIN", c.spreadMin, 4, 64, 4);
    if (const char *t = getenv("XRT_TUNE")) {
        int v[4] = {0, 0, 0, c.tune[3]};
        if (sscanf(t, "%d,%d,%d,%d", &v[0], &v[1], &v[2], &v[3]) >= 3 && v[0] >= 1 && v[0] <= 64 && v[1] >= 1 && v[2] >= 1 && v[3] >= 0 && v[3] <= 64)
            for (int i = 0; i < 4; i++) c.tune[i] = v[i];
    }
    env_int("XRT_HEAVY_SHIFT", c.heavyShift, 0, 6);
    env_int("XRT_FIRST_BATCH", c.firstBatch, 64, 4096, 64);
    env_flag("XRT_PK_MERGE", c.packetMerge);
    env_flag("XRT_AE", c.answerAtEmission);
    env_flag("XRT_AE_FINISH", c.finishInPartA);
    env_flag("XRT_END_EARLY", c.endEarly);
    env_int("XRT_PK_CULL_MIN", c.packetCullMin, INT_MIN, INT_MAX);
    env_flag("XRT_PK_SPLIT", c.packetSplit);
    env_int("XRT_PK_BUDGET", c.packetBudgetUs, 0, 1000000);
    env_int("XRT_PK_BUDGET_ITEM", c.packetBudgetItemUs, 0, 1000000);
    env_int("XRT_PK_SPLIT_ITEMS", c.packetSplitItems, 1, 1 << 20);
    env_int("XRT_PK_LONG", c.packetLongUs, 0, 1000000);
    env_int("XRT_PK_BUDGET_LONG", c.packetBudgetLongUs, 0, 1000000);
    env_int("XRT_PK_GRAB", c.packetGrabMax, 1, 64);
    env_int("XRT_PK_STATIC", c.packetStaticDiv, 0, 64);
    env_flag("XRT_PK_QUADS", c.packetQuads);
    env_flag("XRT_LEVEL_MAP", c.levelMap);
    env_int("XRT_NODE_CULL", c.nodeCull, 0, 2);
    c.noSingle = env_set("XRT_NO_SINGLE");
    if (const char *e = getenv("XRT_LONG_FRAC")) { int lo = 0, hi = 0; if (sscanf(e, "%d,%d", &lo, &hi) == 2 && lo >= 0 && hi > lo && hi <= 100) { c.longFracLo = lo; c.longFracHi = hi; } }
    env_float("XRT_HEAVY", c.heavy);
    env_int("XRT_HEAP_RAY_CAP", c.heapRayCap, 1024, HEAP_RAY_CAP);
    env_int("XRT_SHADOW_BYTES", c.shadowBytes, 1LL << 20, LLONG_MAX);
    env_int("XRT_CHUNK_PATHS", c.maxChunkPaths, 8192, MAX_CHUNK_PATHS, 8192);
    env_int("XRT_PIXEL_BYTES", c.pixelBytes, 1, LLONG_MAX);
    env_float("XRT_OVERLAP_MS", c.overlapMinMs);
    env_int("XRT_SPLIT", c.splitMode, 0, 2);
    env_int("XRT_SPLIT_PARTS", c.splitParts, 2, 4);
    env_float("XRT_SPLIT_MS", c.splitMinMs);
    env_flag("XRT_LAUNCH_EVENTS", c.launchEvents);
    env_int("XRT_STAMP_ROWS", c.maxStampRows, 0, MAX_STAMP_ROWS);
    env_flag("XRT_ADAPTIVE_FAST", c.adaptiveFast);
    env_int("XRT_ADAPTIVE_CAP", c.adaptiveCap, 1, LLONG_MAX);
    env_flag("XRT_HEAP_FAST", c.heapFast);
    env_flag("XRT_GRID_HINTS", c.gridHints);
    env_int("XRT_SHADE_BLOCK", c.shadeBlock, 256, 1024, 64);
    env_flag("XRT_LAUNCH_TIMING", c.launchTiming);
    env_str("XRT_WAVE_TIMES", c.waveTimesPath);
    env_str("XRT_STAMP_DUMP", c.stampDumpPath);
    c.fakeGpus = env_set("XRT_FAKE_GPUS");
    c.noRectCull = env_set("XRT_NO_RECT_CULL"); c.oneStream = env_set("XRT_ONE_STREAM"); c.noFeedback = env_set("XRT_NO_FEEDBACK");
    env_flag("XRT_LEAF_ORDER", c.spatialRuns);
#ifdef XRT_DEV
    if (const char *e = getenv("XRT_LEAF_CULL")) { const double v = atof(e); if (v >= 0.0 && v <= 1e6) c.leafCullSafety = v; }
    if (const char *e = getenv("XRT_CULL_SAFETY")) { const double v = atof(e); if (v >= 0.0 && v <= 1e6) c.cullSafety = v; }
    env_flag("XRT_FINISH_COUNTS", c.finishCounts);
#endif
    env_flag("XRT_GUARD", c.guard);
    return c;
}

}
```

### xna-ray-trace_amd/csrc/xrt_api.cpp

```cpp
#include <hip/hip_runtime.h>

#include <algorithm>
#include <cmath>
#include <cstdio>
#include <cstring>
#include <memory>
#include <mutex>
#include <string>
#include <vector>

#include "../../include/xrt.h"
#include "device_res.h"

using namespace xrt;

#include "scene_state.h"
#include "pixels.h"
#include "pixels_plan.h"
#include "hits.h"
#include "lights.h"
#include "lights_plan.h"
#include "trace.h"
#include "trace_plan.h"
#include "surface.h"
#include "compose.h"

namespace {

bool in_flight(const xrt_scene *s) {
    if (s->busy.load()) return true;
    for (const auto &f : s->frames) if (f.pending) return true;
    return false;
}

int need_device(xrt_scene *s, const char *fn) {
    if (!s) return fail(XRT_E_INVALID_ARG, "%s: null scene", fn);
    if (s->device < 0) return fail(XRT_E_NO_DEVICE, "%s: host-only scene (created with device -1); libxrt has no CPU execution path", fn);
    if (!s->host->built || !s->resident) return fail(XRT_E_NOT_BUILT, "%s: call xrt_scene_build first", fn);
    HIPCHECK(hipSetDevice(s->device));
    return XRT_OK;
}

hipEvent_t get_event(std::vector<Event> &pool, size_t i) {
    while (pool.size() <= i) {
        Event e;
        if (hipEventCreate(&e.h) != hipSuccess) return nullptr;
        pool.push_back(std::move(e));
    }
    return pool[i];
}
hipEvent_t get_event(xrt_scene *s, size_t i) { return get_event(s->events, i); }

ObjRec *pose_objects(xrt_scene *s, int v) { return v == 0 ? s->objects.p : s->pose[v].objects.p; }
f4 *pose_scull(xrt_scene *s, int v) { return v == 0 ? s->scull.p : s->pose[v].scull.p; }
SceneView pose_view(xrt_scene *s, int v) {
    SceneView S = s->view;
    S.objects = pose_objects(s, v); S.scull = pose_scull(s, v);
    return S;
}
int pose_wait(xrt_scene *s, int v, hipStream_t st) {
    if (s->pose[v].ready) HIPCHECK(hipStreamWaitEvent(st, s->pose[v].ready, 0));
    return XRT_OK;
}
int pose_reader(xrt_scene *s, int v, hipStream_t st) {
    auto &rd = s->pose[v].readers;
    size_t i = 0;
    while (i < rd.size() && rd[i].first != st) i++;
    if (i == rd.size()) {
        Event e;
        if (int rc = e.create()) return rc;
        rd.emplace_back(st, std::move(e));
    }
    HIPCHECK(hipEventRecord(rd[i].second, st));
    return XRT_OK;
}
bool pose_referenced(const xrt_scene *s, int v) { return s->slotPose[0] == v || s->slotPose[1] == v; }

DevBuf<MaterialRec> &mat_records(xrt_scene *s, int v) { return v == 0 ? s->materials : s->mat[v].materials; }
// ... 316 lines not shown
        const int shift = 9 + (g.samples == 16 ? 4 : (g.samples == 4 ? 2 : 0));
        const int tx0 = g.cullX0 / XRT_TILE_W, tx1 = g.cullX1 / XRT_TILE_W, ty0 = g.cullY0 / XRT_TILE_H, ty1 = g.cullY1 / XRT_TILE_H;
        const long long kept = (long long)(tx1 - tx0 + 1) * (ty1 - ty0 + 1);
        if (kept < p.totalTiles && (kept << shift) < (long long)p.P) {
            const unsigned inv = (unsigned)(((1ULL << 32) + (unsigned)g.tilesX - 1) / (unsigned)g.tilesX);
            bool exact = p.totalTiles < (1LL << 24);
            if (exact && !(s.lvlCheckedTilesX == g.tilesX && s.lvlCheckedTiles >= p.totalTiles)) {
                for (long long t = 0; exact && t < p.totalTiles; t++) exact = (unsigned)(((unsigned long long)t * inv) >> 32) == (unsigned)(t / g.tilesX);
                p.lvlVerified = exact;
            }
            if (exact) {
                g.lvl.on = 1; g.lvl.tilesX = g.tilesX; g.lvl.tx0 = tx0; g.lvl.ty0 = ty0; g.lvl.rw = tx1 - tx0 + 1; g.lvl.shift = shift; g.lvl.inv = inv;
                p.lvlStride = (size_t)(kept << shift);
            }
        }
    }
    if (heap) {
        const size_t capL = (size_t)std::min<long long>(s.cfg.heapRayCap, lightBound);
        p.rayCap = (R < 20 && ((size_t)p.P << R) < capL) ? ((size_t)p.P << R) : capL;
        if (p.rayCap < (size_t)p.P) p.rayCap = (size_t)p.P;
    }
    if ((unsigned long long)p.rayCap * (unsigned long long)(nL > 0 ? nL : 1) > (1ull << 30)) return fail(XRT_E_UNSUPPORTED, "frame too large: %zu rays x %d lights per generation", p.rayCap, nL);
    p.shadowCap = p.rayCap;
    p.wantF32 = wantsF32 && !adaptive && g.samples == 1;
    p.cntStride = 5 * (R + 2);
    p.qStride = (1 + 2 * PACKET_QUEUE_WORDS) * (R + 2);
    const bool heapOptimistic = heap && heapFastAllowed && s.cfg.heapFast && s.heapFastOk && nParts == 1;
    const bool adaptiveOptimistic = adaptive && !heap && heapFastAllowed && s.cfg.adaptiveFast && s.adaptiveFastOk && nParts == 1 && !p.collect && p.totalPixels * 4 <= p.chunkPaths &&
                                    (p.quality + 2) * (R + 2) * 2 + 2 <= MAX_STAMP_ROWS;
    p.fast = (adaptive ? adaptiveOptimistic : (!heap || heapOptimistic)) && oneChunk && !p.collect && !batch;
    p.heapFast = heapOptimistic && p.fast;
    p.adaptiveFast = adaptiveOptimistic && p.fast;
    if (p.adaptiveFast) {
        p.cntBase = ADAPTIVE_LEVEL_WORDS;
        p.levelCap = (int)(s.cfg.adaptiveCap > 0 ? std::min(s.cfg.adaptiveCap, p.totalPixels) : p.totalPixels);
    }
    p.ae = (p.fast || (batch && oneChunk && !p.collect)) && !heap && !adaptive && nParts == 1 && scene_answers_at_emission(s);
    p.finishA = p.ae && !p.capturePaths && nL <= 32 && s.cfg.finishInPartA;
    p.endEarly = p.finishA && p.fast && !wantsF32 && s.cfg.endEarly;
    p.skipTiles = p.endEarly && g.lvl.on != 0 && g.samples > 1;
    p.endSkipped = p.skipTiles ? (unsigned long long)(p.totalTiles - lvl_kept_tiles(g)) << g.lvl.shift : 0;
    p.fuseResolve = !adaptive && !heap && !batch && g.samples == 1 && !p.endEarly;
    p.useStamps = !s.cfg.launchEvents && s.cfg.launchTiming && s.wallClockKHz > 0;
    p.ownStream = !hasStream && p.fast && s.lastFrameMs >= s.cfg.overlapMinMs && !s.cfg.oneStream;
    p.tileCosts = p.fast && !adaptive && !heap && s.packetOk && p.framePaths < (1LL << 31);
    const int pkSamples = (batch && batch->coherent) ? batch->samples : g.samples;
    const int pkHeap = s.cfg.packetMaskHeap >= 0 ? s.cfg.packetMaskHeap : ((s.sceneMode == MODE_SCENE && (long long)g.width * g.height * g.samples >= 600000LL) ? 7 : 0);
    const int pkScene = heap ? (s.packetOk ? pkHeap : 0) : scene_packet_mask(s, pkSamples);
    p.pkMask = (batch && !batch->coherent && (heap ? s.cfg.packetMaskHeap : s.cfg.packetMask) < 0) ? (pkScene & ~1) : pkScene;
    if (s.cfg.packetQuads && (p.pkMask & 1) && (!batch || (batch->coherent && batch->gen))) {
        const long long walk = p.skipTiles ? ((long long)lvl_kept_tiles(g) << g.lvl.shift) : (long long)p.P;
        p.pkEntries = (size_t)((walk + 63) / 64);
    }
    const bool laneClosest = (p.pkMask & 5) != 5;
    p.wantFeedback = p.fast && !heap && !adaptive && s.deepMeshes && !s.cfg.noFeedback && laneClosest;
    p.listLong = s.heavyPath > 0.0f || p.wantFeedback;
    p.hinted = p.fast && nParts == 1 && s.genKey == firstPaths * 64 + nL && s.genHeap == heap && s.cfg.gridHints;
    p.shadeBlock = s.cfg.shadeBlock;
    if (batch) p.validPixels = (unsigned long long)batch->n;
    else {
        const long long slot0 = p.partStart / (512LL * g.samples), slot1 = (p.partStart + firstPaths + 512LL * g.samples - 1) / (512LL * g.samples);
        for (long long sl = slot0; sl < slot1; sl++) {
            const long long t = tile_of_slot(s, p, sl);
            if (t >= p.totalTiles) break;
            if (t < 0) continue;
            const int tx = (int)(t % g.tilesX), ty = (int)(t / g.tilesX);
            const int w = std::min(g.width - tx * XRT_TILE_W, (int)XRT_TILE_W), h = std::min(g.height - ty * XRT_TILE_H, (int)XRT_TILE_H);
            p.validPixels += (unsigned long long)w * h;
        }
    }
    if (int rc = lights_known(nullptr, lights, nL)) return rc;
    plan = p;
    return XRT_OK;
}

namespace {

int frame_finish(xrt_scene *s, xrt_scene::FrameCtx &F, xrt_stats *stats);
int split_arena(xrt_scene *s, DevBuf<unsigned> &items, DevBuf<unsigned> &recs, PacketArgs &PA, hipStream_t st);

static inline long long gen_hits(const int *hc, int R, int k) { return (long long)hc[(R + 2) + k] + (long long)hc[4 * (R + 2) + k]; }

void tally_chunk(xrt_scene::FrameCtx &F, const int *hc) {
    const FramePlan &P = F.plan;
    const int R = P.R;
    for (int k = 0; k <= R; k++) {
        F.shaded += (unsigned long long)gen_hits(hc, R, k);
        if (k > 0) F.closestDeep += (unsigned long long)(P.heap ? hc[k] : gen_hits(hc, R, k - 1));
        else F.live0 += (unsigned long long)hc[0];
        if (P.ae) {
            F.answered += (unsigned long long)gen_hits(hc, R, k) * (unsigned long long)P.nL - (unsigned long long)hc[3 * (R + 2) + k];
            if (k < R) F.answered += (unsigned long long)(gen_hits(hc, R, k) - hc[k + 1]);
        }
    }
}

int ensure_frame_buffers(xrt_scene *s, xrt_scene::FrameCtx &F, const FramePlan &P, unsigned &freshPathRecs) {
    xrt_scene::WorkBufs &W = F.w;
    const size_t rayCap = P.rayCap, perLight = rayCap * (size_t)(P.nL > 0 ? P.nL : 1);
    int rc;
    if ((rc = W.rays0.ensure(rayCap)) || (rc = W.rays1.ensure(rayCap)) || (rc = W.hits.ensure(rayCap)) || (rc = W.path0.ensure(rayCap)) ||
        (rc = W.path1.ensure(rayCap)) || (rc = W.hitFlags0.ensure(rayCap)) ||
        (rc = W.shadowFlags.ensure(perLight)) || (rc = W.slot0.ensure(rayCap)) ||
        (rc = W.slot1.ensure(rayCap)) || (rc = W.index0.ensure(rayCap)) || (rc = W.heavyList.ensure(rayCap)) || (rc = W.shadowRays.ensure(perLight)) ||
        (rc = W.shadowHits.ensure(perLight)) || (rc = W.lvlA.ensure(P.lvlStride * P.nodes)) ||
        (rc = W.lvlB.ensure(P.lvlStride * P.nodes)) || (rc = W.sampleColor.ensure(P.P)) || (rc = W.lights.ensure(P.nL > 0 ? P.nL : 1)) ||
        (rc = s->counters.ensure(2 * C_COUNT + 8)))
        return rc;
    if (!s->cfg.waveTimesPath.empty() && !s->waveTimes.p) {
        if ((rc = s->waveTimes.ensure((size_t)16 * 3 * 8192))) return rc;
        HIPCHECK(hipMemset(s->waveTimes.p, 0, (size_t)16 * 3 * 8192 * sizeof(unsigned long long)));
    }
    if (P.heap && ((rc = W.node0.ensure(rayCap)) || (rc = W.node1.ensure(rayCap)) || (rc = W.ref0.ensure(rayCap)) || (rc = W.ref1.ensure(rayCap)) ||
                   (rc = W.slotNode0.ensure(rayCap)) || (rc = W.slotNode1.ensure(rayCap)) ||
                   (rc = W.lvlAlpha.ensure((size_t)P.P * P.nodes))))
        return rc;
    if (P.wantF32 && !P.batch && (rc = W.sampleF32.ensure((size_t)P.P * 3))) return rc;
    if (P.ae && ((rc = W.shadowOut.ensure(perLight)) || (rc = W.shadowFlags1.ensure(perLight)))) return rc;
    if (P.endEarly) {
        const int *before = W.composeList.p;
        if ((rc = W.composeList.ensure(rayCap + 16))) return rc;
        if (W.composeList.p != before) {
            HIPCHECK(hipMemsetAsync(W.composeList.p, 0, 16 * sizeof(int), s->stream));
            HIPCHECK(hipStreamSynchronize(s->stream));
        }
    }
    if (P.pkEntries) {
        const unsigned *before = W.quadTable.p; const size_t capBefore = W.quadTable.cap;
        if ((rc = W.quadTable.ensure((size_t)QUAD_HEAD_WORDS + 2 * P.pkEntries))) return rc;
        if (W.quadTable.p != before || W.quadTable.cap != capBefore) {
            HIPCHECK(hipMemsetAsync(W.quadTable.p, 0, QUAD_HEAD_WORDS * sizeof(unsigned), s->stream));
            HIPCHECK(hipStreamSynchronize(s->stream));
        }
    }
    if (P.useStamps) {
        if ((rc = W.stamps.ensure((size_t)MAX_STAMP_ROWS * STAMP_STRIDE))) return rc;
        if ((rc = F.stampHost.ensure((size_t)MAX_STAMP_ROWS * 2 * sizeof(unsigned long long), hipHostMallocMapped))) return rc;
    }
    freshPathRecs = 0;
    if (P.capturePaths) {
        auto ensure_fresh = [&](DevBuf<f4> &b, size_t n, unsigned bit) -> int {
            const f4 *before = b.p; const size_t capBefore = b.cap;
            const int rc2 = b.ensure(n);
            if (rc2 == XRT_OK && (b.p != before || b.cap != capBefore)) freshPathRecs |= bit;
            return rc2;
        };
        const size_t pathBlocks = ((size_t)P.P + PATHS_BLOCK - 1) / PATHS_BLOCK;
        if ((rc = ensure_fresh(s->pathHit, P.lvlStride * P.nodes, 1u)) || (P.heap && (rc = ensure_fresh(s->pathDir, P.lvlStride * P.nodes, 2u))) || (rc = s->pathLocal.ensure((size_t)P.P)) ||
            (rc = s->pathBlockSum.ensure(pathBlocks)) || (rc = s->pathBlockBase.ensure(pathBlocks)))
            return rc;
        if ((rc = s->pathPinned.ensure(64, hipHostMallocDefault))) return rc;
    }
    return XRT_OK;
}

struct ChunkPost {
    enum Kind { NOTHING, EMIT_PATHS, RESOLVE, COPY_LEVEL } kind = NOTHING;
    uint32_t *levelColor = nullptr;
};

struct FrameJob {
    xrt_scene *s;
    xrt_scene::FrameCtx &F;
    const FramePlan &P;
    xrt_scene::WorkBufs &W;
    SceneView S;
    ShadeView V;
    hipStream_t st;
    hipEvent_t e0, e1;
    const BatchSrc *batch;
    uint32_t *d_out;
    float *d_outF32;
    unsigned *tileCostDev;
    int *overflowFlag;
    bool startEvent;
    unsigned pathEpoch = 0;

    static constexpr int QW = 1 + 2 * PACKET_QUEUE_WORDS;

    struct Step {
        const RayGenParams &gp;
        unsigned *q;
        long long pathBase;
        int k;
        const int *pathOfClosest;
        const SlotRec *slotPrev;
    };

    bool packet_closest(int k) const { const int m = P.pkMask; return (k == 0 ? (m & 1) : (k == 1 ? (m & 4) : ((m & 4) && (m & 16)))) != 0; }
    bool packet_shadow(int k) const { return (P.pkMask & 2) != 0 && (k <= 1 || (P.pkMask & 16) != 0); }
    long long hint(const long long *v, int k) const { return (P.hinted && k < 68 && v[k] >= 0) ? 4 * v[k] + 4096 : -1; }
    int ensure_pinned(size_t bytes) { return F.pinned.bytes < bytes ? F.pinned.ensure(bytes + 4096, hipHostMallocMapped) : XRT_OK; }
    HeavyArgs heavy_for(int k, int *hcnt) const;
    int pick_timing(int grid, unsigned long long *&stamps, hipEvent_t &a0, hipEvent_t &a1);
    int launch_packets(const Step &T, const IntersectArgs &I, bool shadow, long long nHost, const IntersectArgs *I2 = nullptr, const QuadTable *quads = nullptr);
    int launch_lanes(const Step &T, const IntersectArgs *C, const IntersectArgs *B, int Pc);
    int enqueue_chunk(const RayGenParams &gp, int *cnt, unsigned *q, int Pc, long long pathBase, uint32_t *sampleOut = nullptr, const FrameEpilogue *epi = nullptr,
                      int *listCnt = nullptr);
    int post_chunk(const ChunkPost &post, int Pc, long long pathBase);
    int run_pass_tree(const RayGenParams &gp, long long total, const ChunkPost &post, float progress0, float progress1, bool finalPass);
    int run_pass(const RayGenParams &gp, long long total, const ChunkPost &post, float progress0, float progress1, bool finalPass);
    int batch_frame();
    int plain_frame();
    int adaptive_in_flight();
    int adaptive_careful();
};

HeavyArgs FrameJob::heavy_for(int k, int *hcnt) const {
    HeavyArgs H;
    if (P.listLong && (k == 0 || !P.heap) && !packet_closest(k)) {
        H.list = W.heavyList.p; H.count = hcnt + k; H.path = s->heavyPath;
        if (P.wantFeedback) { H.costMap = s->costMap.p + (size_t)k * (size_t)P.framePaths + (size_t)P.partStart; H.epoch = s->epoch & 0xffffu; H.costThreshold = s->costT[k]; }
    }
    return H;
}

int FrameJob::pick_timing(int grid, unsigned long long *&stamps, hipEvent_t &a0, hipEvent_t &a1) {
    a0 = get_event(F.events, F.ev); a1 = get_event(F.events, F.ev + 1);
    if (!a0 || !a1) return fail(XRT_E_HIP, "hipEventCreate failed");
    if (P.useStamps && grid * 4 <= STAMP_SLOTS && F.stampRows < s->cfg.maxStampRows) { stamps = W.stamps.p + (size_t)F.stampRows++ * STAMP_STRIDE; a0 = a1 = nullptr; }
    else if (!s->cfg.launchTiming) a0 = a1 = nullptr;
    else { F.pairs.push_back({F.ev, F.ev + 1}); F.ev += 2; }
    return XRT_OK;
}

int FrameJob::launch_packets(const Step &T, const IntersectArgs &I, bool shadow, long long nHost, const IntersectArgs *I2, const QuadTable *quads) {
    const int k = T.k, word = shadow ? 1 : 0, R = P.R, nL = P.nL;
    int rc;
    PacketArgs PA = packet_args(s, I, I2, quads);
    PA.queue += PACKET_QUEUE_WORDS * word;
    if (tileCostDev) {
        PA.tileCost = tileCostDev; PA.tileBase = (int)T.pathBase; PA.tileShift = 9 + (T.gp.samples == 16 ? 4 : (T.gp.samples == 4 ? 2 : 0));
        if (shadow) { PA.slotOf1 = T.slotPrev; PA.nL1 = nL; }
        else PA.pathOf1 = T.pathOfClosest;
        if (I2) { PA.slotOf2 = T.slotPrev; PA.nL2 = nL; }
    }
    if (s->cfg.packetSplit && s->sceneMode != MODE_SCENE) {
        if ((rc = split_arena(s, W.splitItems, W.splitRecs, PA, st))) return rc;
        if (P.fast && !P.adaptive && !P.heap && s->cfg.packetLongUs > 0) {
            const size_t stride = std::max((P.rayCap + 63) / 64, P.pkEntries) + ((size_t)P.shadowCap * (size_t)(nL > 0 ? nL : 1) + 63) / 64 + 2;
            if (W.splitCostStride != stride || !W.splitCost.p) {
                if ((rc = W.splitCost.ensure(stride * 2 * (size_t)(R + 2)))) return rc;
                HIPCHECK(hipMemsetAsync(W.splitCost.p, 0, stride * 2 * (size_t)(R + 2) * sizeof(unsigned), st));
                W.splitCostStride = stride;
            }
            PA.splitCost = W.splitCost.p + stride * (size_t)(2 * k + word);
            PA.splitLong = s->cfg.packetLongUs; PA.splitBudgetLong = std::max(1, s->cfg.packetBudgetLongUs);
        }
    }
    const int grid = packet_grid(s, s->blocksPerCUPacket, nHost);
    hipEvent_t a0, a1;
    if ((rc = pick_timing(grid, PA.stamps, a0, a1))) return rc;
    launch_packet(S, PA, grid, st, a0, a1);
    return XRT_OK;
}

int FrameJob::launch_lanes(const Step &T, const IntersectArgs *C, const IntersectArgs *B, int Pc) {
    const int k = T.k;
    IntersectArgs A = C ? *C : *B;
    if (C && B) { A.rays2 = B->rays; A.hits2 = B->hits; A.flags2 = B->flags; A.nDev2 = B->nDev; A.nMul2 = B->nMul; A.nCap2 = B->nCap; A.scatter2 = B->scatter; }
    const int grid = k == 0 ? persistent_grid(s, Pc) : persistent_grid(s, hint(s->genRays, k), 16);
    hipEvent_t a0, a1;
    if (int rc = pick_timing(grid, A.stamps, a0, a1)) return rc;
    if (s->waveTimes.p && k < 16) A.debugTimes = s->waveTimes.p + (size_t)k * 3 * 8192;
    launch_intersect(S, A, s->stackNeeded, grid, st, a0, a1);
    return XRT_OK;
}

int FrameJob::enqueue_chunk(const RayGenParams &gp, int *cnt, unsigned *q, int Pc, long long pathBase, uint32_t *sampleOut, const FrameEpilogue *epi, int *listCnt) {
    const int R = P.R, nL = P.nL;
    const bool heap = P.heap, ae = P.ae, fast = P.fast, feedback = P.wantFeedback;
    const size_t rayCap = P.rayCap, shadowCap = P.shadowCap;
    int rc;
    int *scnt = cnt + (R + 2), *hcnt = cnt + 2 * (R + 2), *acnt = cnt + 3 * (R + 2);
    int *fcnt = cnt + 4 * (R + 2);
    const int chunkRow0 = F.stampRows;
    if (P.capturePaths) {
        if (++s->pathEpoch == 0) {
            HIPCHECK(hipMemsetAsync(s->pathHit.p, 0, s->pathHit.cap * sizeof(f4), st));
            if (s->pathDir.p) HIPCHECK(hipMemsetAsync(s->pathDir.p, 0, s->pathDir.cap * sizeof(f4), st));
            s->pathEpoch = 1;
        }
        pathEpoch = s->pathEpoch;
    }
    xrt_ray *rays[2] = {W.rays0.p, W.rays1.p};
    int *paths[2] = {W.path0.p, W.path1.p};
    int *nodesOf[2] = {W.node0.p, W.node1.p};
    float *refOf[2] = {W.ref0.p, W.ref1.p};
    RayGenParams gb = gp;
    if (P.batch && heap) gb.batchRef = refOf[0];
    EndArgs endArgs;
    if (listCnt) {
        endArgs.on = 1; endArgs.sampleColor = sampleOut ? sampleOut : W.sampleColor.p;
        endArgs.list = W.composeList.p + 16; endArgs.cnt = listCnt; endArgs.listCap = (int)rayCap;
        endArgs.skipTiles = P.skipTiles ? 1 : 0;
    }
    QuadTable quads;
    if (P.pkEntries && (!P.batch || batch->gen) && gp.quadLevel <= 0 && packet_closest(0) && (P.skipTiles || ((size_t)Pc + 63) / 64 <= P.pkEntries)) {
        W.quadWord ^= 1;
        quads.table = reinterpret_cast<uint2 *>(W.quadTable.p + QUAD_HEAD_WORDS); quads.cap = (int)P.pkEntries;
        quads.count = W.quadTable.p + 64 * W.quadWord; quads.clear = W.quadTable.p + 64 * (W.quadWord ^ 1);
    }
    if (P.givenHits) {
        Range r("xrt ingest hits");
        IngestHitsArgs G;
        G.rays = batch->rays; G.hits = batch->hits; G.pathBase = pathBase; G.P = Pc;
        G.raysOut = rays[0]; G.hitsOut = W.hits.p; G.flagsOut = W.hitFlags0.p; G.index = W.index0.p; G.count = cnt; G.lvlB0 = W.lvlB.p;
        G.refOut = heap ? refOf[0] : nullptr; G.refIndex = batch->refIndex; G.liveCap = (int)rayCap;
        launch_ingest_hits(S, G, st, startEvent ? e0 : nullptr);
        startEvent = false;
    } else if (P.batch && batch->gen) {
        Range r("xrt pixel raygen");
        launch_pixel_raygen(*batch->gen, S, rays[0], W.lvlB.p, W.index0.p, cnt, Pc, pathBase, heavy_for(0, hcnt), (int)rayCap, heap ? refOf[0] : nullptr, batch->refIndex, quads, st,
                            startEvent ? e0 : nullptr);
        startEvent = false;
    } else
    { Range r("xrt raygen"); launch_raygen(gb, S, rays[0], W.lvlB.p, W.index0.p, cnt, Pc, pathBase, heavy_for(0, hcnt), st, startEvent ? e0 : nullptr, (int)rayCap, &endArgs, &quads); startEvent = false; }
    xrt_hit *hitsOf[2] = {W.hits.p, W.hits.p};
    int *flagsOf[2] = {W.hitFlags0.p, W.hitFlags0.p};
    SlotRec *slotOf[2] = {W.slot0.p, W.slot1.p};
    int *slotNodeOf[2] = {W.slotNode0.p, W.slotNode1.p};
    int *const shadowFlagsOf[2] = {W.shadowFlags.p, ae ? W.shadowFlags1.p : W.shadowFlags.p};
    for (int k = 0; k <= R + 1; k++) {
        const int cur = k & 1, prv = cur ^ 1;
        const bool hasClosest = k <= R, hasShadow = k >= 1 && nL > 0;
        const bool traceClosest = hasClosest && !(k == 0 && P.givenHits);
        const int *nClosest = (k == 0 || heap || ae) ? cnt + k : scnt + (k - 1);
        IntersectArgs C, B;
        C.rays = rays[cur]; C.hits = hitsOf[cur]; C.index = nullptr; C.nDev = nClosest; C.nMul = 1; C.n = Pc;
        C.nCap = (int)rayCap;
        C.flags = flagsOf[cur]; B.flags = shadowFlagsOf[(k + 1) & 1];
        C.missRecords = (feedback && !packet_closest(k)) ? 1 : 0;
        { const HeavyArgs H = heavy_for(k, hcnt); C.heavyIdx = H.list; C.nHeavy = H.count; }
        B.rays = W.shadowRays.p; B.hits = W.shadowHits.p; B.index = nullptr; B.nDev = hasShadow ? scnt + (k - 1) : nullptr; B.nMul = nL; B.n = 0;
        if (ae && hasShadow) { B.nDev = acnt + (k - 1); B.nMul = 1; B.scatter = W.shadowOut.p; }
        B.nCap = (int)((long long)shadowCap * nL);
        for (IntersectArgs *a : {&C, &B}) {
            a->queue = q + QW * k; a->mode = s->sceneMode; a->meshId = 0;
            set_knobs(*a, s);
        }
        const bool pkC = traceClosest && packet_closest(k), pkB = hasShadow && packet_shadow(k);
        const Step T{gp, q, pathBase, k, k == 0 ? W.index0.p : paths[cur], slotOf[prv]};
        Range ri("xrt intersect #%d", k);
        if (pkC && pkB && s->cfg.packetMerge) { if ((rc = launch_packets(T, C, false, hint(s->genRays, k), &B))) return rc; }
        else {
            if (pkC && (rc = launch_packets(T, C, false, k == 0 ? Pc : hint(s->genRays, k), nullptr, k == 0 ? &quads : nullptr))) return rc;
            if (pkB && (rc = launch_packets(T, B, true, hint(s->genRays, k)))) return rc;
        }
        const bool laneC = traceClosest && !pkC, laneB = hasShadow && !pkB;
        if ((laneC || laneB) && (rc = launch_lanes(T, laneC ? &C : nullptr, laneB ? &B : nullptr, Pc))) return rc;
        if ((hasClosest || hasShadow) && P.collect) {
            if (traceClosest) launch_count(S, C, s->counters.p, st);
            if (hasShadow) launch_count(S, B, s->counters.p + C_COUNT, st);
        }
        if (ri.on) { roctx().pop(); ri.on = false; }
        Range rs("xrt shade #%d", k);
        ShadeArgs X;
        std::memset(&X, 0, sizeof(X));
        X.level = k; X.doA = hasClosest ? 1 : 0; X.doB = k >= 1 ? 1 : 0;
        X.maxReflections = R; X.P = (int)P.lvlStride; X.lvl = gp.lvl; X.heap = heap ? 1 : 0; X.overflow = overflowFlag;
        X.rays = rays[cur]; X.hits = hitsOf[cur]; X.hitFlags = flagsOf[cur]; X.shadowFlags = shadowFlagsOf[(k + 1) & 1]; X.nDev = nClosest; X.nHost = Pc; X.cap = (int)rayCap;
        X.index = nullptr; X.rayPath = k == 0 ? W.index0.p : paths[cur];
        X.rayNode = (heap && k > 0) ? nodesOf[cur] : nullptr;
        X.rayRef = (heap && (k > 0 || P.batch)) ? refOf[cur] : nullptr;
        X.slotOut = slotOf[cur]; X.slotNodeOut = heap ? slotNodeOf[cur] : nullptr; X.scnt = scnt + k; X.shadowCap = (int)shadowCap; X.shadowRays = W.shadowRays.p;
        X.nextRays = rays[prv]; X.nextPath = paths[prv]; X.nextNode = heap ? nodesOf[prv] : nullptr; X.nextRef = heap ? refOf[prv] : nullptr;
        X.nextCnt = cnt + k + 1; X.nextCap = (int)rayCap;
        if (ae) { X.ae = 1; X.shadowCnt = acnt + k; X.shadowOut = W.shadowOut.p; X.shadowFlagsOut = shadowFlagsOf[k & 1]; }
        if (P.finishA) { X.finish = 1; X.finishCnt = fcnt + k; }
        if (listCnt && k == 0) X.end = endArgs;
// ... 1222 lines not shown
        if (!hinted) {
            if (!raysOut) listRays = W.rays.p;
            launch_pixel_rays(G.cam, G.cx, G.cy, G.stride, G.first, (int)m, G.size, G.mode, raysOut ? raysOut : W.rays.p, st);
            HIPCHECK(hipGetLastError());
            if (hitsOut) {
                std::lock_guard<std::mutex> lock(s->apiMutex);
                if ((rc = run_intersect(s, listRays, P, hitsOut, s->sceneMode, 0, st, nullptr, false, W.ev[2], W.ev[3]))) return rc;
                traced = true;
            }
        } else {
            HIPCHECK(hipMemsetAsync(W.queue.p, 0, (1 + PACKET_QUEUE_WORDS) * sizeof(unsigned), st));
            QuadTable Q;
            if (table) {
                xrt_scene::WorkBufs &FW = F0.w;
                FW.quadWord ^= 1;
                Q.table = reinterpret_cast<uint2 *>(FW.quadTable.p + QUAD_HEAD_WORDS); Q.cap = (int)tableCap;
                Q.count = FW.quadTable.p + 64 * FW.quadWord; Q.clear = FW.quadTable.p + 64 * (FW.quadWord ^ 1);
            }
            launch_trace_raygen(G, S, raysOut, hitsOut, W.rays.p, F0.w.index0.p, W.counts.p, P, P, Q, st);
            IntersectArgs A = IntersectArgs();
            A.rays = W.rays.p; A.hits = hitsOut; A.index = nullptr; A.nDev = W.counts.p; A.nMul = 1; A.n = P; A.nCap = P;
            A.queue = W.queue.p; A.mode = s->sceneMode; A.meshId = 0;
            A.flags = nullptr; A.missRecords = 0; A.scatter = F0.w.index0.p;
            if ((rc = launch_list_traversal(s, S, A, packets, &Q, W.splitItems, W.splitRecs, P, st, W.ev[2], W.ev[3]))) return rc;
            traced = true;
            if (collect && !listRays) {
                launch_pixel_rays(G.cam, G.cx, G.cy, G.stride, G.first, (int)m, G.size, G.mode, W.countRays.p, st);
                listRays = W.countRays.p;
            }
        }
        if (hitsOut && stats) launch_trace_hits(hitsOut, P, W.counts.p + 1, st);
        if (collect) {
            IntersectArgs K = IntersectArgs();
            K.rays = listRays; K.hits = nullptr; K.index = nullptr; K.nDev = nullptr; K.nMul = 1; K.n = P; K.nCap = 0; K.queue = nullptr; K.mode = s->sceneMode; K.meshId = 0;
            set_knobs(K, s);
            launch_count(S, K, s->counters.p, st);
        }
        HIPCHECK(hipGetLastError());
        HIPCHECK(hipEventRecord(W.ev[1], st));
        int hc[2] = {0, 0};
        HIPCHECK(hipMemcpyAsync(hc, W.counts.p, sizeof(hc), hipMemcpyDeviceToHost, st));
        HIPCHECK(hipStreamSynchronize(st));
        if (hinted && (hc[0] < 0 || hc[0] > P)) return fail(XRT_E_INTERNAL, "xrt_trace_pixels: %d live rays in a chunk of %d places", hc[0], P);
        live += hitsOut ? (hinted ? (unsigned long long)hc[0] : (unsigned long long)P) : 0ull;
        found += (unsigned long long)hc[1];
        float ms = 0.0f;
        HIPCHECK(hipEventElapsedTime(&ms, W.ev[0], W.ev[1]));
        msTotal += ms;
        if (traced) {
            HIPCHECK(hipEventElapsedTime(&ms, W.ev[2], W.ev[3]));
            msIntersect += ms; msLongest = std::max(msLongest, (double)ms); launches++;
        }
        if (table && b.size() == 2) {
            F0.plan.pkEntries = tableCap;
            s->quadCtx = 0; s->quadLive = (unsigned long long)hc[0];
        }
    }
    if (stats) {
        std::memset(stats, 0, sizeof(*stats));
        if (collect) {
            unsigned long long hcnt[2 * C_COUNT];
            HIPCHECK(hipMemcpy(hcnt, s->counters.p, sizeof(hcnt), hipMemcpyDeviceToHost));
            fill_stats(stats, hcnt, 0, (unsigned long long)n);
        }
        stats->pixels = (uint64_t)n;
        stats->rays_closest = d_hits ? (uint64_t)n * (uint64_t)samples : 0;
        stats->hits_closest = found;
        stats->rays_traversed = live;
        stats->ms_total = msTotal; stats->ms_intersect = msIntersect; stats->ms_intersect_longest = msLongest; stats->intersect_launches = launches;
    }
    return XRT_OK;
}

int light_hits_impl(xrt_scene *s, const xrt_hit *d_hits, int64_t n, const xrt_light *lights, int32_t nL, float *d_light, float *d_amount, hipStream_t st,
                    xrt_stats *stats) {
    xrt_scene::LightWork &W = s->lightWork;
    int rc;
    const std::vector<long long> b = light_chunks(n, nL, (uint64_t)s->cfg.shadowBytes);
    const size_t pairsCap = (size_t)(b[1] - b[0]) * (size_t)nL;
    if ((rc = W.counts.ensure(4))) return rc;
    if (nL > 0 && ((rc = W.rays.ensure(pairsCap)) || (rc = W.hits.ensure(pairsCap)) || (rc = W.flags.ensure(pairsCap)) || (rc = W.scatter.ensure(pairsCap)) ||
                   (rc = W.queue.ensure(1 + PACKET_QUEUE_WORDS)) || (rc = W.lights.ensure((size_t)nL))))
        return rc;
    for (Event &e : W.ev) if ((rc = e.create(hipEventDefault))) return rc;
    const int pv = s->poseCur, mv = s->matCur, sv = s->shadeCur;
    if ((rc = pose_wait(s, pv, st)) || (rc = mat_acquire(s, mv, st)) || (rc = shade_wait(s, sv, st))) return rc;
    std::vector<LightRec> hl((size_t)(nL > 0 ? nL : 1));
    for (int i = 0; i < nL; i++) hl[(size_t)i] = make_light(lights[i]);
    if (nL > 0) HIPCHECK(hipMemcpyAsync(W.lights.p, hl.data(), (size_t)nL * sizeof(LightRec), hipMemcpyHostToDevice, st));
    const SceneView S = pose_view(s, pv);
    ShadeView V = shade_view(s, mv, sv);
    V.lights = W.lights.p; V.nLights = nL;
    const bool ae = scene_answers_at_emission(*s);
    const bool packets = (scene_packet_mask(*s, 1) & 2) != 0;
    unsigned long long live = 0, traced = 0;
    double msTotal = 0.0, msIntersect = 0.0;
    unsigned launches = 0;
    Range rf("xrt light hits");
    for (size_t c = 0; c + 1 < b.size(); c++) {
        const int m = (int)(b[c + 1] - b[c]);
        HIPCHECK(hipMemsetAsync(W.counts.p, 0, 4 * sizeof(int), st));
        HIPCHECK(hipEventRecord(W.ev[0], st));
        if (nL > 0) {
            HIPCHECK(hipMemsetAsync(W.queue.p, 0, (1 + PACKET_QUEUE_WORDS) * sizeof(unsigned), st));
            LightEmitArgs E;
            E.hits = d_hits; E.base = b[c]; E.n = m; E.nLights = nL; E.lights = W.lights.p; E.ae = ae ? 1 : 0;
            E.rays = W.rays.p; E.scatter = W.scatter.p; E.flags = W.flags.p; E.count = W.counts.p; E.cap = (int)((size_t)m * (size_t)nL);
// ... 916 lines not shown
    if (rank_stride < 0 || (rank_stride > 0 && rank_stride < (int64_t)tiles_per_rank * 512)) return fail(XRT_E_INVALID_ARG, "xrt_detile_table_device: rank_stride smaller than a rank's tiles");
    launch_detile(width, height, shard_count, tiles_per_rank, (const uint32_t *)d_gathered, rank_stride > 0 ? rank_stride : (long long)tiles_per_rank * 512,
                  (uint32_t *)d_rgba_out, (hipStream_t)stream, (const int *)d_tile_of_slot);
    HIPCHECK(hipGetLastError());
    return XRT_OK;
}

int xrt_rccl_probe(void) {
    return guarded("xrt_rccl_probe", [&]() -> int {
        RcclGather g;
        std::string err;
        if (!g.probe(err)) return fail(XRT_E_RCCL, "%s", err.c_str());
        return XRT_OK;
    });
}

float xrt_progress(const xrt_scene *scene) { return scene ? scene->progress.load() : 0.0f; }

int xrt_debug_end_counts(xrt_scene *scene, uint64_t out[3]) {
    return guarded("xrt_debug_end_counts", [&]() -> int {
        int rc = need_device(scene, "xrt_debug_end_counts");
        if (rc != XRT_OK) return rc;
        if (!out) return fail(XRT_E_INVALID_ARG, "xrt_debug_end_counts: null argument");
        for (int i = 0; i < 3; i++) out[i] = scene->endCounts[i];
        return XRT_OK;
    });
}

int xrt_debug_packet_table(xrt_scene *scene, uint64_t counts[2], uint32_t *entries_out, int64_t entries_cap, int32_t *paths_out, int64_t paths_cap) {
    return guarded("xrt_debug_packet_table", [&]() -> int {
        int rc = need_device(scene, "xrt_debug_packet_table");
        if (rc != XRT_OK) return rc;
        if (!counts || entries_cap < 0 || paths_cap < 0 || (!entries_out && entries_cap > 0) || (!paths_out && paths_cap > 0))
            return fail(XRT_E_INVALID_ARG, "xrt_debug_packet_table: null argument or negative capacity");
        BusyGuard guard(scene);
        if (!guard.owned || scene->frames[0].pending || scene->frames[1].pending) return fail(XRT_E_BUSY, "Current render operation not finished.");
        counts[0] = counts[1] = 0;
        if (scene->quadCtx < 0) return XRT_OK;
        const xrt_scene::WorkBufs &W = scene->frames[scene->quadCtx].w;
        const FramePlan &P = scene->frames[scene->quadCtx].plan;
        HIPCHECK(hipSetDevice(scene->device));
        HIPCHECK(hipDeviceSynchronize());
        unsigned n = 0;
        HIPCHECK(hipMemcpy(&n, W.quadTable.p + 64 * W.quadWord, sizeof(n), hipMemcpyDeviceToHost));
        if ((size_t)n > P.pkEntries) return fail(XRT_E_INTERNAL, "xrt_debug_packet_table: %u entries in a table sized for %zu", n, P.pkEntries);
        counts[0] = n; counts[1] = scene->quadLive;
        const size_t ne = std::min<size_t>(n, (size_t)entries_cap), np = std::min<size_t>((size_t)scene->quadLive, (size_t)paths_cap);
        if (ne) HIPCHECK(hipMemcpy(entries_out, W.quadTable.p + QUAD_HEAD_WORDS, ne * 2 * sizeof(uint32_t), hipMemcpyDeviceToHost));
        if (np) HIPCHECK(hipMemcpy(paths_out, W.index0.p, np * sizeof(int32_t), hipMemcpyDeviceToHost));
        return XRT_OK;
    });
}

int xrt_split_stats(xrt_scene *scene, uint64_t out[4], int32_t reset) {
    return guarded("xrt_split_stats", [&]() -> int {
        int rc = need_device(scene, "xrt_split_stats");
        if (rc != XRT_OK) return rc;
        if (!out) return fail(XRT_E_INVALID_ARG, "xrt_split_stats: null argument");
        unsigned long long v[4] = {0, 0, 0, 0};
        HIPCHECK(hipSetDevice(scene->device));
        HIPCHECK(hipDeviceSynchronize());
        if (packet_split_stats(v, reset != 0) != 0) return fail(XRT_E_HIP, "xrt_split_stats: %s", hipGetErrorString(hipGetLastError()));
        for (int i = 0; i < 4; i++) out[i] = v[i];
        return XRT_OK;
    });
}

}

namespace {

template <class F>
int list_call(const char *fn, const xrt_scene *scene, F &&body) {
    return guarded(fn, [&]() -> int { return scene ? body(fn) : fail(XRT_E_INVALID_ARG, "%s: null scene", fn); });
}

bool empty_list(int64_t n, xrt_stats *stats) {
    if (stats) std::memset(stats, 0, sizeof(*stats));
    return n == 0;
}

int hits_name_scene(const char *fn, const xrt_scene *scene, const xrt_hit *hits, int64_t n, bool withBody) {
    const auto &meshes = scene->host->meshes; const auto &bodies = scene->host->objects;
    for (int64_t i = 0; i < n; i++) {
        const xrt_hit &h = hits[i];
        if (h.hit == 0) continue;
        if (h.mesh < 0 || h.mesh >= (int)meshes.size()) return fail(XRT_E_INVALID_ARG, "%s: hit %lld names mesh %d, which does not exist", fn, (long long)i, h.mesh);
        if (h.tri < 0 || h.tri >= meshes[(size_t)h.mesh].ntri)
            return fail(XRT_E_INVALID_ARG, "%s: hit %lld names triangle %d of mesh %d, which does not exist", fn, (long long)i, h.tri, h.mesh);
        if (!withBody) continue;
        if (h.object < 0 || h.object >= (int)bodies.size()) return fail(XRT_E_INVALID_ARG, "%s: hit %lld names body %d, which does not exist", fn, (long long)i, h.object);
        const std::vector<int> &bm = bodies[(size_t)h.object].meshes;
        if (std::find(bm.begin(), bm.end(), h.mesh) == bm.end())
            return fail(XRT_E_INVALID_ARG, "%s: hit %lld names mesh %d, which is not a mesh of body %d", fn, (long long)i, h.mesh, h.object);
    }
    return XRT_OK;
}

int rays_name_scene(const char *fn, const xrt_scene *scene, const xrt_ray *rays, int64_t n) {
    const auto &meshes = scene->host->arrays.meshes;
    for (int64_t i = 0; i < n; i++) {
        const xrt_ray &r = rays[i];
        if (r.ignore_tri < 0) continue;
        if (r.ignore_mesh < 0 || r.ignore_mesh >= (int)meshes.size() || r.ignore_tri >= meshes[(size_t)r.ignore_mesh].ntri)
            return fail(XRT_E_INVALID_ARG, "%s: ray %lld names triangle %d of mesh %d, which does not exist", fn, (long long)i, r.ignore_tri, r.ignore_mesh);
    }
// ... 479 lines not shown
```

Before: 18840.

## Cull packet leaf triangles by precomputed screen-space rectangles

Adds a per-frame pass that projects every triangle reference into a quantised screen rectangle, and records a screen rectangle per ray packet during ray generation. In single-mesh packet traversal, each leaf's triangles are ballot-tested against the packet's rectangle, and only overlapping triangles are intersected via a bitmask iteration. This aims to cut triangle tests that cannot be hit by primary-ray packets. It costs an extra kernel over all references each frame, extra memory, and branchier leaf loops. It also changes launch bounds for the single-mode kernel, which may affect occupancy.

```diff
diff --git a/include/xrt.h b/include/xrt.h
--- a/include/xrt.h
+++ b/include/xrt.h
@@ -215,6 +215,8 @@
 
 int xrt_debug_packet_table(xrt_scene *scene, uint64_t counts[2], uint32_t *entries_out, int64_t entries_cap, int32_t *paths_out, int64_t paths_cap);
 
+int xrt_debug_screen_table(xrt_scene *scene, int32_t host_eval, uint64_t *count, uint32_t *entries_out, int64_t entries_cap);
+
 float xrt_progress(const xrt_scene *scene);
 
 int xrt_generate_primary_rays(xrt_scene *scene, const xrt_camera *camera, xrt_ray *rays_out );
diff --git a/xna-ray-trace_amd/_abi.py b/xna-ray-trace_amd/_abi.py
--- a/xna-ray-trace_amd/_abi.py
+++ b/xna-ray-trace_amd/_abi.py
@@ -140,6 +140,7 @@
     "xrt_split_stats": (C.c_int, [C.c_void_p, _P(C.c_uint64), C.c_int32]),
     "xrt_debug_end_counts": (C.c_int, [C.c_void_p, _P(C.c_uint64)]),
     "xrt_debug_packet_table": (C.c_int, [C.c_void_p, _P(C.c_uint64), _P(C.c_uint32), C.c_int64, _P(C.c_int32), C.c_int64]),
+    "xrt_debug_screen_table": (C.c_int, [C.c_void_p, C.c_int32, _P(C.c_uint64), _P(C.c_uint32), C.c_int64]),
     "xrt_generate_primary_rays": (C.c_int, [C.c_void_p, _P(xrt_camera), _P(xrt_ray)]),
     "xrt_cast_rays": (C.c_int, [C.c_void_p, _P(xrt_ray), C.c_int64, C.c_int32, C.c_float, _P(xrt_light), C.c_int32, _P(xrt_render_opts),
                                 _P(C.c_uint32), _F, _P(xrt_stats)]),
diff --git a/xna-ray-trace_amd/api.py b/xna-ray-trace_amd/api.py
--- a/xna-ray-trace_amd/api.py
+++ b/xna-ray-trace_amd/api.py
@@ -516,6 +516,14 @@
                                                    paths.ctypes.data_as(C.POINTER(C.c_int32)), paths.shape[0]))
         return entries, paths
 
+    def ScreenTable(self, host_eval=False):
+        count = C.c_uint64(0)
+        abi.check(abi.lib().xrt_debug_screen_table(self.handle, 1 if host_eval else 0, C.byref(count), None, 0))
+        entries = np.zeros((int(count.value), 2), dtype=np.uint32)
+        if entries.shape[0]:
+            abi.check(abi.lib().xrt_debug_screen_table(self.handle, 1 if host_eval else 0, C.byref(count), entries.ctypes.data_as(C.POINTER(C.c_uint32)), entries.shape[0]))
+        return entries
+
     def IntersectBatch(self, rays, stats=False):
         rays = np.ascontiguousarray(rays, dtype=RAY_DTYPE)
         hits = np.zeros(rays.shape[0], dtype=HIT_DTYPE)
diff --git a/xna-ray-trace_amd/csrc/frame_plan.h b/xna-ray-trace_amd/csrc/frame_plan.h
--- a/xna-ray-trace_amd/csrc/frame_plan.h
+++ b/xna-ray-trace_amd/csrc/frame_plan.h
@@ -63,6 +63,7 @@
     bool useStamps = false;
     int pkMask = 0;
     size_t pkEntries = 0;
+    size_t scrRefs = 0;
     int shadeBlock = 1024;
     bool ownStream = false;
     int cntBase = 0, levelCap = 0;
diff --git a/xna-ray-trace_amd/csrc/kernels.h b/xna-ray-trace_amd/csrc/kernels.h
--- a/xna-ray-trace_amd/csrc/kernels.h
+++ b/xna-ray-trace_amd/csrc/kernels.h
@@ -93,12 +93,17 @@
     const uint2 *pkTable = nullptr;
     const unsigned *pkCount = nullptr;
     int pkCap = 0;
+    const uint2 *scrTable = nullptr;
+    const uint2 *pkRect = nullptr;
 };
 struct QuadTable {
     uint2 *table = nullptr;
     unsigned *count = nullptr, *clear = nullptr;
     int cap = 0;
-};
+    uint2 *rect = nullptr;
+};
+constexpr int SCREEN_XF_SLOTS = 64;
+void launch_screen_rects(const RayGenParams &g, const ObjRec *objects, const float *refT, int nRefs, uint2 *table, hipStream_t st);
 constexpr int QUAD_HEAD_WORDS = 128;
 constexpr int PACKET_QUEUE_HEADS = 8, PACKET_HEAD_STRIDE = 64;
 constexpr int PACKET_SPLIT_WORDS = 320;
diff --git a/xna-ray-trace_amd/csrc/kernels.hip b/xna-ray-trace_amd/csrc/kernels.hip
--- a/xna-ray-trace_amd/csrc/kernels.hip
+++ b/xna-ray-trace_amd/csrc/kernels.hip
@@ -1,6 +1,7 @@
 #include "kernels.h"
 #include "device_util.h"
 #include "pose.h"
+#include "screen_rects.h"
 #include "shade_math.h"
 
 #include <hip/hip_ext.h>
@@ -590,7 +591,19 @@
         if (wave == 0 && Q.table) reserve_cells_and_entries(ldsLive, count, Q.count, quadLen, quadAt);
         else if (wave < 2 && (wave == 0 || H.list)) reserve_cells(wave == 0 ? ldsLive : ldsHeavy, wave == 0 ? count : H.count);
         __syncthreads();
-        if (quadLen > 0 && quadAt < Q.cap) Q.table[quadAt] = make_uint2((unsigned)ldsLive[lane], (unsigned)quadLen);
+        if (quadLen > 0 && quadAt < Q.cap) {
+            Q.table[quadAt] = make_uint2((unsigned)ldsLive[lane], (unsigned)quadLen);
+            if (Q.rect) {
+                const int q0 = grp * span + (lane >> 4) * APPEND_BLOCK + (lane & 15) * 64;
+                int p0 = q0;
+                if constexpr (END) { if (keptWalk) p0 = lvl_walk_path(g.lvl, (unsigned)q0 >> g.lvl.shift, (unsigned)q0); }
+                const int sshift = g.samples == 16 ? 4 : (g.samples == 4 ? 2 : 0);
+                int x = 0, y = 0;
+                (void)path_pixel(g, (pathBase + p0) >> sshift, x, y);
+                const ScrEntry e = screen_packet_rect(x, y, g.samples == 16 ? 2 : (g.samples == 4 ? 4 : 8), g.quadLevel >= 0 ? 4 : (g.samples == 16 ? 6 : 0));
+                Q.rect[quadAt] = make_uint2(e.x, e.y);
+            }
+        }
 #pragma unroll
         for (int r = 0; r < RG_ROUNDS; r++) {
             const int p = path_of(grp * span + r * APPEND_BLOCK + (int)threadIdx.x);
diff --git a/xna-ray-trace_amd/csrc/packet.hip b/xna-ray-trace_amd/csrc/packet.hip
--- a/xna-ray-trace_amd/csrc/packet.hip
+++ b/xna-ray-trace_amd/csrc/packet.hip
@@ -1,5 +1,6 @@
 #include "device_util.h"
 #include "kernels.h"
+#include "screen_rects.h"
 
 #include <hip/hip_ext.h>
 
@@ -178,7 +179,7 @@
     }
 };
 
-template <bool SPLIT, bool LEAF_RHO>
+template <bool SPLIT, bool LEAF_RHO, bool SCR>
 __device__ __forceinline__ void pk_walk(const float *__restrict__ pblocks, const float *__restrict__ refT, const float *__restrict__ lrec,
                                         const SceneView &S, int cullMin, unsigned *stk, int lane, Lane &L,
                                         const RayCull &RC, bool fastL, int rootBlock, unsigned long long lanes0, bool nodeCull,
@@ -320,14 +321,31 @@
             PKC(3);
             const f4 *const nr = reinterpret_cast<const f4 *>(lrec + (size_t)node * LREC_WORDS);
             const f4 nlo = nr[0], nhi = nr[1];
+            int r0 = 0, r1 = 0;
+            auto leaf_refs = [&]() {
+                const unsigned long long offLo = (unsigned long long)(unsigned)f2i(B.w[4]) | ((unsigned long long)(unsigned)f2i(B.w[5]) << 32);
+                const unsigned long long offHi = (unsigned long long)(unsigned)f2i(B.w[6]) | ((unsigned long long)(unsigned)f2i(B.w[7]) << 32);
+                r0 = d1 + child_ref_offset(offLo, offHi, c);
+                r1 = d1 + ((c == 7) ? d3 : child_ref_offset(offLo, offHi, c + 1));
+            };
+            unsigned long long keepM = ~0ull;
+            if constexpr (SCR) {
+                leaf_refs();
+                const Frame4 sw = *reinterpret_cast<const Frame4 *>(sst + 8);
+                const unsigned long long tp = (unsigned long long)(unsigned)rfl((int)sw.c) | ((unsigned long long)(unsigned)rfl((int)sw.d) << 32);
+                {
+                    const bool mineE = lane < r1 - r0;
+                    uint2 e = make_uint2(0u, 0u);
+                    if (mineE) e = reinterpret_cast<const uint2 *>(tp)[r0 + lane];
+                    keepM = __ballot(mineE && screen_overlap(e.x, e.y, sw.a, sw.b));
+                }
+            }
             bool go = inC & !all_back_facing(nlo, nhi, L.r.d);
             if (keyed) go = go & !((L.mfound != 0) & (key > L.mKey));
             if (!__any(go)) continue;
+            if constexpr (SCR) { if (keepM == 0ull && r1 - r0 <= 64) continue; }
             PKC(4);
-            const unsigned long long offLo = (unsigned long long)(unsigned)f2i(B.w[4]) | ((unsigned long long)(unsigned)f2i(B.w[5]) << 32);
-            const unsigned long long offHi = (unsigned long long)(unsigned)f2i(B.w[6]) | ((unsigned long long)(unsigned)f2i(B.w[7]) << 32);
-            const int r0 = d1 + child_ref_offset(offLo, offHi, c);
-            const int r1 = d1 + ((c == 7) ? d3 : child_ref_offset(offLo, offHi, c + 1));
+            if constexpr (!SCR) leaf_refs();
             const bool big = r1 - r0 >= LEAF_RUN_MIN;
             float rho = 0.0f;
             bool usable = false;
@@ -346,12 +364,21 @@
             PKC(5);
             int nRuns = 1, rb = -1;
             if (big) { rb = f2i(lrec[(size_t)node * LREC_WORDS + 24]); if (rb >= 0) nRuns = (r1 - r0 + LEAF_RUN - 1) / LEAF_RUN; }
+            if constexpr (SCR) { if (rb < 0) nRuns = (r1 - r0 + 63) >> 6; }
             const bool cheap = LEAF_RHO && !__any(go && !usable);
             for (int jr = 0; jr < nRuns; jr++) {
                 int ra = r0, rz = r1;
                 bool goR = go;
+                unsigned long long m = ~0ull;
+                if constexpr (SCR) {
+                    const int runLen = rb >= 0 ? LEAF_RUN : 64;
+                    ra = r0 + runLen * jr; rz = min(ra + runLen, r1);
+                    m = ra - r0 < 64 ? keepM >> (ra - r0) : ~0ull;
+                    if (rz - ra < 64) m &= (1ull << (rz - ra)) - 1ull;
+                    if (m == 0ull) continue;
+                }
                 if (rb >= 0) {
-                    ra = r0 + LEAF_RUN * jr; rz = min(ra + LEAF_RUN, r1);
+                    if constexpr (!SCR) { ra = r0 + LEAF_RUN * jr; rz = min(ra + LEAF_RUN, r1); }
                     const f4 *tb = reinterpret_cast<const f4 *>(lrec + (size_t)rb + (size_t)jr * RUN_WORDS);
                     PKC(6);
                     if (cheap) goR = go && !grown_box_missed(L.r, tb[0], tb[1], rho);
@@ -361,8 +388,11 @@
                 }
                 PKC(7);
 #ifdef XRT_PK_COUNTERS
-                pkc[8] += (unsigned)(rz - ra);
-                pkc[14] += (unsigned)(rz - ra) * (unsigned)__popcll(__ballot(goR));
+                {
+                    const unsigned steps = SCR ? (unsigned)__popcll(m) : (unsigned)(rz - ra);
+                    pkc[8] += steps;
+                    pkc[14] += steps * (unsigned)__popcll(__ballot(goR));
+                }
 #endif
                 if (goR) {
                     L.leafKey = key; L.leafNode = node;
@@ -377,6 +407,25 @@
                             }
                         }
                     };
+                    if constexpr (SCR) {
+                        int j0 = (int)__builtin_ctzll(m);
+                        m &= m - 1ull;
+                        TriWords qA = *reinterpret_cast<const TriWords *>(pt + j0 * TRI_REC_BYTES);
+                        for (;;) {
+                            const bool more1 = m != 0ull;
+                            const int j1 = more1 ? (int)__builtin_ctzll(m) : j0;
+                            m &= m - 1ull;
+                            const TriWords qB = *reinterpret_cast<const TriWords *>(pt + j1 * TRI_REC_BYTES);
+                            test(qA, ra + j0);
+                            if (!more1) break;
+                            const bool more0 = m != 0ull;
+                            j0 = more0 ? (int)__builtin_ctzll(m) : j1;
+                            m &= m - 1ull;
+                            qA = *reinterpret_cast<const TriWords *>(pt + j0 * TRI_REC_BYTES);
+                            test(qB, ra + j1);
+                            if (!more0) break;
+                        }
+                    } else {
                     TriWords qA = *reinterpret_cast<const TriWords *>(pt);
                     int r = ra;
                     for (;;) {
@@ -387,6 +436,7 @@
                         test(qB, r + 1);
                         r += 2; pt += 2 * TRI_REC_BYTES;
                         if (r >= rz) break;
+                    }
                     }
                 }
             }
@@ -449,7 +499,7 @@
 #define PK_SCENE_WAVES 5
 #endif
 template <int M, bool SP>
-__global__ __launch_bounds__(256, (M == MODE_SCENE) ? PK_SCENE_WAVES : (PK_SINGLE_WAVES >= 7 ? 7 : (SP ? 6 : 1))) __attribute__((amdgpu_num_sgpr(PK_SGPRS))) void k_packet(const float *__restrict__ pblocks, const float *__restrict__ refT,
+__global__ __launch_bounds__(256, (M == MODE_SCENE) ? PK_SCENE_WAVES : (PK_SINGLE_WAVES >= 7 ? 7 : 6)) __attribute__((amdgpu_num_sgpr(PK_SGPRS))) void k_packet(const float *__restrict__ pblocks, const float *__restrict__ refT,
                                                 const float *__restrict__ lrec, const MeshRec *__restrict__ meshes,
                                                 const f4 *__restrict__ snodes, const f4 *__restrict__ scull, const ObjRec *__restrict__ objects,
                                                 const int *__restrict__ objMesh, SceneView S, PacketArgs A) {
@@ -621,7 +671,23 @@
                     __builtin_amdgcn_fence(__ATOMIC_ACQUIRE, "wavefront");
                 }
             }
-            pk_walk<splitOn, true>(pblocks, refT, lrec, S, A.cullMin, stk, lane, L, RC, fastL, mr.rootBlock, lanes0, nodeCull, splitOn && item >= 0);
+            bool scr = false;
+            if constexpr (!splitOn) {
+                KA.fresh();
+                scr = !seg2 && KA.args()->scrTable != nullptr && KA.args()->pkTable != nullptr;
+                if (scr) {
+                    if (lane == 0) {
+                        const uint2 rc = KA.args()->pkRect[pk];
+                        const unsigned long long tp = (unsigned long long)KA.args()->scrTable;
+                        *reinterpret_cast<Frame4 *>(sst + 8) = Frame4{rc.x, rc.y, (unsigned)tp, (unsigned)(tp >> 32)};
+                    }
+                    __builtin_amdgcn_fence(__ATOMIC_RELEASE, "wavefront");
+                    __builtin_amdgcn_wave_barrier();
+                    __builtin_amdgcn_fence(__ATOMIC_ACQUIRE, "wavefront");
+                }
+            }
+            if (scr) pk_walk<false, true, true>(pblocks, refT, lrec, S, A.cullMin, stk, lane, L, RC, fastL, mr.rootBlock, lanes0, nodeCull, false);
+            else pk_walk<splitOn, true, false>(pblocks, refT, lrec, S, A.cullMin, stk, lane, L, RC, fastL, mr.rootBlock, lanes0, nodeCull, splitOn && item >= 0);
             L.mesh = mesh;
             KA.fresh();
             bool mine = true;
@@ -780,7 +846,7 @@
                                 const bool meshAway = nodeCull && mesh_faces_away(mr, L.r.d);
                                 const unsigned long long lanes0 = __ballot(inRoot && !meshAway);
                                 if (lanes0 != 0ull)
-                                    pk_walk<false, false>(pblocks, refT, lrec, S, A.cullMin, stk, lane, L, RC, fastL, rootBlock, lanes0, nodeCull, false);
+                                    pk_walk<false, false, false>(pblocks, refT, lrec, S, A.cullMin, stk, lane, L, RC, fastL, rootBlock, lanes0, nodeCull, false);
                             }
                             if (L.mfound) {
                                 L.mesh = m; C.obj = o;
diff --git a/xna-ray-trace_amd/csrc/scene_state.h b/xna-ray-trace_amd/csrc/scene_state.h
--- a/xna-ray-trace_amd/csrc/scene_state.h
+++ b/xna-ray-trace_amd/csrc/scene_state.h
@@ -188,6 +188,7 @@
         DevBuf<int> path0, path1, index0, heavyList, cnts;
         DevBuf<int> composeList;
         DevBuf<unsigned> quadTable;
+        DevBuf<uint2> scrTable, pkRect;
         int quadWord = 0;
         DevBuf<int> node0, node1, heapFlag;
         DevBuf<float> ref0, ref1, lvlAlpha;
diff --git a/xna-ray-trace_amd/csrc/screen_rects.h b/xna-ray-trace_amd/csrc/screen_rects.h
--- /dev/null
+++ b/xna-ray-trace_amd/csrc/screen_rects.h
@@ -0,0 +1,269 @@
+#pragma once
+#include "xrt_core.h"
+
+namespace xrt {
+
+constexpr unsigned SCR_NO_CULL = 0xffffffffu;
+constexpr int SCR_UNITS = 16, SCR_BIAS = 8, SCR_MAX = 65534;
+constexpr int SCR_MAX_EXTENT = 4000;
+struct ScrEntry { unsigned x, y; };
+
+struct ScreenXf {
+    double F[16];
+    double E[3];
+    double vpX, vpY, vpW, vpH;
+    double dN;
+    double epsO;
+    double epsT;
+    double fx, fy, fw;
+    double resid;
+    int ok;
+    int why;
+};
+
+XRT_HD bool scr_invert4(const double *B, double *F) {
+    double a[4][8];
+#pragma unroll
+    for (int i = 0; i < 4; i++) {
+#pragma unroll
+        for (int j = 0; j < 4; j++) { a[i][j] = B[4 * i + j]; a[i][4 + j] = i == j ? 1.0 : 0.0; }
+    }
+    bool ok = true;
+#pragma unroll
+    for (int c = 0; c < 4; c++) {
+#pragma unroll
+        for (int r = c + 1; r < 4; r++) {
+            const bool sw = fabs(a[r][c]) > fabs(a[c][c]);
+#pragma unroll
+            for (int j = 0; j < 8; j++) { const double t = a[r][j], w = a[c][j]; a[c][j] = sw ? t : w; a[r][j] = sw ? w : t; }
+        }
+        ok = ok && fabs(a[c][c]) > 0.0;
+        const double inv = 1.0 / a[c][c];
+#pragma unroll
+        for (int j = 0; j < 8; j++) a[c][j] *= inv;
+#pragma unroll
+        for (int r = 0; r < 4; r++) {
+            if (r == c) continue;
+            const double f = a[r][c];
+#pragma unroll
+            for (int j = 0; j < 8; j++) a[r][j] -= f * a[c][j];
+        }
+    }
+#pragma unroll
+    for (int i = 0; i < 4; i++) {
+#pragma unroll
+        for (int j = 0; j < 4; j++) F[4 * i + j] = a[i][4 + j];
+    }
+    return ok;
+}
+XRT_HD void scr_mul4(const double *a, const double *b, double *r) {
+    for (int i = 0; i < 4; i++)
+        for (int j = 0; j < 4; j++) r[4 * i + j] = a[4 * i] * b[j] + a[4 * i + 1] * b[4 + j] + a[4 * i + 2] * b[8 + j] + a[4 * i + 3] * b[12 + j];
+}
+XRT_HD bool scr_point(const double *M, double X, double Y, double Z, double *p) {
+    double v[4];
+    for (int j = 0; j < 4; j++) v[j] = X * M[j] + Y * M[4 + j] + Z * M[8 + j] + M[12 + j];
+    if (!(fabs(v[3]) > 1e-300)) return false;
+    p[0] = v[0] / v[3]; p[1] = v[1] / v[3]; p[2] = v[2] / v[3];
+    return true;
+}
+
+XRT_HD void make_screen_xf(const RayGenParams &g, const float *invWorld, ScreenXf &X) {
+    const double u = 5.9604644775390625e-8;
+    X.ok = 0; X.why = 1; X.resid = 0.0;
+    X.vpX = g.vpX; X.vpY = g.vpY; X.vpW = g.vpW; X.vpH = g.vpH;
+    double G[16], IW[16], B[16];
+#pragma unroll
+    for (int i = 0; i < 16; i++) { G[i] = g.m[i]; IW[i] = invWorld[i]; }
+    IW[3] = 0.0; IW[7] = 0.0; IW[11] = 0.0; IW[15] = 1.0;
+    scr_mul4(G, IW, B);
+    if (!scr_invert4(B, X.F)) return;
+    X.why = 2;
+    {
+        double I[16];
+        scr_mul4(B, X.F, I);
+#pragma unroll
+        for (int i = 0; i < 16; i++) { const double d = fabs(I[i] - ((i % 5) == 0 ? 1.0 : 0.0)); if (!(d <= 1e-6)) return; X.resid = fmax(X.resid, d); }
+    }
+    X.why = 3;
+    if (!(fabs(B[11]) > 1e-9 * (fabs(B[8]) + fabs(B[9]) + fabs(B[10])))) return;
+#pragma unroll
+    for (int j = 0; j < 3; j++) X.E[j] = B[8 + j] / B[11];
+    X.why = 4;
+    if (!(g.vpW > 0.0f && g.vpH > 0.0f) || !(fabs((double)g.depthRange) > 0.0)) return;
+    X.why = 5;
+    const double sxs[5] = {-1.0, (double)g.width, -1.0, (double)g.width, 0.5 * g.width}, sys[5] = {-1.0, -1.0, (double)g.height, (double)g.height, 0.5 * g.height};
+    const double Zs[2] = {(0.0 - (double)g.minDepth) / (double)g.depthRange, (1.0 - (double)g.minDepth) / (double)g.depthRange};
+    double Xm = 0.0, Ym = 0.0, aMin[2] = {1e300, 1e300}, pMax[2] = {0.0, 0.0}, vMax[2][4] = {{0.0, 0.0, 0.0, 0.0}, {0.0, 0.0, 0.0, 0.0}}, lMin = 1e300, dN = 0.0, oAx[3] = {0.0, 0.0, 0.0};
+    double pws[5][2][3];
+    int aSign = 0;
+#pragma unroll
+    for (int c = 0; c < 5; c++) {
+        const double Xc = ((sxs[c] - X.vpX) / X.vpW) * 2.0 - 1.0, Yc = -(((sys[c] - X.vpY) / X.vpH) * 2.0 - 1.0);
+        Xm = fmax(Xm, fabs(Xc)); Ym = fmax(Ym, fabs(Yc));
+        double (&pw)[2][3] = pws[c], pb[3];
+#pragma unroll
+        for (int z = 0; z < 2; z++) {
+            const double a = Xc * G[3] + Yc * G[7] + Zs[z] * G[11] + G[15];
+            const int sg = a > 0.0 ? 1 : (a < 0.0 ? -1 : 0);
+            if (sg == 0 || (aSign != 0 && sg != aSign)) return;
+            aSign = sg;
+            aMin[z] = fmin(aMin[z], fabs(a));
+#pragma unroll
+            for (int j = 0; j < 4; j++) vMax[z][j] = fmax(vMax[z][j], fabs(Xc * G[j] + Yc * G[4 + j] + Zs[z] * G[8 + j] + G[12 + j]));
+            if (!scr_point(G, Xc, Yc, Zs[z], pw[z])) return;
+            pMax[z] = fmax(pMax[z], sqrt(pw[z][0] * pw[z][0] + pw[z][1] * pw[z][1] + pw[z][2] * pw[z][2]));
+        }
+#pragma unroll
+        for (int j = 0; j < 3; j++) oAx[j] = fmax(oAx[j], fabs(pw[0][j]));
+        if (!scr_point(B, Xc, Yc, Zs[0], pb)) return;
+        const double ex = pb[0] - X.E[0], ey = pb[1] - X.E[1], ez = pb[2] - X.E[2];
+        dN = fmax(dN, sqrt(ex * ex + ey * ey + ez * ez));
+    }
+    double eP[2];
+#pragma unroll
+    for (int z = 0; z < 2; z++) {
+        double eC[4];
+        const bool zExact = Zs[z] == 0.0 || Zs[z] == 1.0;
+#pragma unroll
+        for (int j = 0; j < 4; j++) {
+            const double tx = Xm * fabs(G[j]), ty = Ym * fabs(G[4 + j]), tz = fabs(Zs[z]) * fabs(G[8 + j]);
+            double e = (u * tx + 4.0 * u * fabs(G[j])) + (u * ty + 4.0 * u * fabs(G[4 + j])) + (zExact ? 0.0 : 5.0 * u * tz);
+            if (tx > 0.0 && ty > 0.0) e += u * (tx + ty);
+            if (tx + ty > 0.0 && tz > 0.0) e += u * (tx + ty + tz);
+            e += u * vMax[z][j];
+            eC[j] = 1.01 * e;
+        }
+        const double eNum = sqrt(eC[0] * eC[0] + eC[1] * eC[1] + eC[2] * eC[2]);
+        eP[z] = 1.1 * (eNum + pMax[z] * eC[3]) / aMin[z] + 4.0 * u * pMax[z];
+    }
+    {
+        const double *n0 = pws[0][0], *n1 = pws[1][0], *n2 = pws[2][0];
+        const double a1[3] = {n1[0] - n0[0], n1[1] - n0[1], n1[2] - n0[2]}, a2[3] = {n2[0] - n0[0], n2[1] - n0[1], n2[2] - n0[2]};
+        const double nn[3] = {a1[1] * a2[2] - a1[2] * a2[1], a1[2] * a2[0] - a1[0] * a2[2], a1[0] * a2[1] - a1[1] * a2[0]};
+        const double nl = sqrt(nn[0] * nn[0] + nn[1] * nn[1] + nn[2] * nn[2]);
+        int sg = 0;
+#pragma unroll
+        for (int c = 0; c < 5 && nl > 0.0; c++) {
+            const double *f = pws[c][1];
+            const double d = (nn[0] * (f[0] - n0[0]) + nn[1] * (f[1] - n0[1]) + nn[2] * (f[2] - n0[2])) / nl;
+            const int sd = d > 0.0 ? 1 : (d < 0.0 ? -1 : 0);
+            if (sd == 0 || (sg != 0 && sd != sg)) { lMin = 0.0; break; }
+            sg = sd;
+            lMin = fmin(lMin, 0.999 * fabs(d));
+        }
+        if (!(nl > 0.0) || lMin > 1e299) lMin = 0.0;
+    }
+    X.why = 6;
+    if (!(lMin > 0.0)) return;
+    const double epsTW = 1.1 * (eP[0] + eP[1]) / lMin + 8.0 * u;
+    double eV2 = 0.0, oN2 = 0.0;
+#pragma unroll
+    for (int j = 0; j < 3; j++) {
+        const double cj = 3.1 * u * ((oAx[0] + eP[0] + 1.0) * fabs(IW[j]) + (oAx[1] + eP[0] + 1.0) * fabs(IW[4 + j]) + (oAx[2] + eP[0] + 1.0) * fabs(IW[8 + j]) + fabs(IW[12 + j]));
+        eV2 += cj * cj;
+        oN2 += (oAx[j] + eP[0] + 1.0) * (oAx[j] + eP[0] + 1.0);
+    }
+    const double eV = sqrt(eV2), oM = sqrt(oN2);
+    const double c00 = IW[5] * IW[10] - IW[6] * IW[9], c01 = IW[6] * IW[8] - IW[4] * IW[10], c02 = IW[4] * IW[9] - IW[5] * IW[8];
+    const double det = IW[0] * c00 + IW[1] * c01 + IW[2] * c02;
+    X.why = 7;
+    if (!(fabs(det) > 1e-300)) return;
+    const double inv3[9] = {c00 / det, (IW[2] * IW[9] - IW[1] * IW[10]) / det, (IW[1] * IW[6] - IW[2] * IW[5]) / det,
+                            c01 / det, (IW[0] * IW[10] - IW[2] * IW[8]) / det, (IW[2] * IW[4] - IW[0] * IW[6]) / det,
+                            c02 / det, (IW[1] * IW[8] - IW[0] * IW[9]) / det, (IW[0] * IW[5] - IW[1] * IW[4]) / det};
+    double n1 = 0.0, nInf = 0.0, i1 = 0.0, iInf = 0.0;
+#pragma unroll
+    for (int k = 0; k < 3; k++) {
+        n1 = fmax(n1, fabs(IW[k]) + fabs(IW[4 + k]) + fabs(IW[8 + k])); nInf = fmax(nInf, fabs(IW[4 * k]) + fabs(IW[4 * k + 1]) + fabs(IW[4 * k + 2]));
+        i1 = fmax(i1, fabs(inv3[k]) + fabs(inv3[3 + k]) + fabs(inv3[6 + k])); iInf = fmax(iInf, fabs(inv3[3 * k]) + fabs(inv3[3 * k + 1]) + fabs(inv3[3 * k + 2]));
+    }
+    const double op = sqrt(n1 * nInf), lb = 1.0 / sqrt(i1 * iInf);
+    X.epsO = op * eP[0] + eV;
+    X.epsT = 1.1 * (2.0 * eV + op * (epsTW + 1.01 * u * oM)) / lb + 8.0 * u;
+    X.dN = dN + X.epsO;
+    const double all = X.dN + X.epsO + X.epsT + fabs(X.E[0]) + fabs(X.E[1]) + fabs(X.E[2]);
+    X.why = 8;
+    if (!(all < 1e30) || !(X.epsT < 1e-2)) return;
+    X.why = 9;
+    if (g.width > SCR_MAX_EXTENT || g.height > SCR_MAX_EXTENT) return;
+    X.fx = 1.000001 * sqrt(X.F[0] * X.F[0] + X.F[4] * X.F[4] + X.F[8] * X.F[8]);
+    X.fy = 1.000001 * sqrt(X.F[1] * X.F[1] + X.F[5] * X.F[5] + X.F[9] * X.F[9]);
+    X.fw = 1.000001 * sqrt(X.F[3] * X.F[3] + X.F[7] * X.F[7] + X.F[11] * X.F[11]);
+    if (!(X.fx + X.fy + X.fw < 1e30)) return;
+    X.ok = 1; X.why = 0;
+}
+
+XRT_HD ScrEntry screen_entry(const ScreenXf &X, const float *v1, const float *E1, const float *E2) {
+    const ScrEntry none = {SCR_NO_CULL, SCR_NO_CULL};
+    if (!X.ok) return none;
+    const float u = 5.9604645e-8f;
+    const float N[3] = {E1[1] * E2[2] - E1[2] * E2[1], E1[2] * E2[0] - E1[0] * E2[2], E1[0] * E2[1] - E1[1] * E2[0]};
+    const float nn = sqrt_rn((N[0] * N[0] + N[1] * N[1]) + N[2] * N[2]);
+    const float l1 = sqrt_rn((E1[0] * E1[0] + E1[1] * E1[1]) + E1[2] * E1[2]), l2 = sqrt_rn((E2[0] * E2[0] + E2[1] * E2[1]) + E2[2] * E2[2]);
+    const float eMax = fmaxf(l1, l2), eMin = fminf(l1, l2);
+    if (!(eMin >= 1e-9f && eMax <= 1e12f) || !(nn > 1e-6f * (l1 * l2))) return none;
+    const float A = 1.0001f * (l1 * l2) / nn;
+    const float Ef[3] = {(float)X.E[0], (float)X.E[1], (float)X.E[2]};
+    float T[3][3], R2 = 0.0f;
+    for (int k = 0; k < 3; k++) {
+        for (int j = 0; j < 3; j++) T[k][j] = (v1[j] + (k == 1 ? E1[j] : (k == 2 ? E2[j] : 0.0f))) - Ef[j];
+        R2 = fmaxf(R2, (T[k][0] * T[k][0] + T[k][1] * T[k][1]) + T[k][2] * T[k][2]);
+    }
+    const float eyeAbs = (fabsf(Ef[0]) + fabsf(Ef[1])) + fabsf(Ef[2]);
+    const float R = 1.0001f * sqrt_rn(R2) + 4.0f * u * (eyeAbs + eMax);
+    const float dNf = 1.0001f * (float)X.dN;
+    const float h = fabsf((N[0] * T[0][0] + N[1] * T[0][1]) + N[2] * T[0][2]) / nn;
+    const float hMin = 0.9999f * h - dNf - 16.0f * u * (R + eyeAbs), tMax = R + dNf;
+    if (!(hMin > 0.0f)) return none;
+    const float cosLB = (0.429f * hMin * nn / eMax - 1.001f * u * (10.5f * eMax * tMax + 8.8f * eMax * eMax)) / (1.001f * (eMax * tMax + 1.01f * nn));
+    const float c0 = fminf(0.5f, cosLB);
+    if (!(c0 > 0.0f) || !(17.4f * u * A / c0 <= 0.5f)) return none;
+    const float rhoC = 126.0f * u * (A / c0) * (tMax + eMax);
+    const float c1 = fmaxf(c0, 0.9999f * hMin / (tMax + rhoC + 2.0f * u * eMax));
+    const float rho = 126.0f * u * (A / c1) * (tMax + eMax);
+    const float deltaF = 1.02f * (rho + 2.0f * u * eMax + (float)X.epsO + (tMax + rho) * (float)X.epsT);
+    if (!(deltaF < 1e30f)) return none;
+    const double delta = deltaF;
+    double sxMin = 1e300, sxMax = -1e300, syMin = 1e300, syMax = -1e300, wMin = 1e300, padF = 0.0;
+    for (int k = 0; k < 3; k++) {
+        double p[3], v[4];
+        for (int j = 0; j < 3; j++) p[j] = (double)v1[j] + (k == 1 ? (double)E1[j] : (k == 2 ? (double)E2[j] : 0.0));
+        for (int j = 0; j < 4; j++) v[j] = p[0] * X.F[j] + p[1] * X.F[4 + j] + p[2] * X.F[8 + j] + X.F[12 + j];
+        const double scale = fabs(v[0]) + fabs(v[1]) + fabs(v[2]) + fabs(v[3]);
+        if (!(v[3] > 1e-3 * scale) || !(scale < 1e30)) return none;
+        const double rw = (double)(1.0f / (float)v[3]);
+        const double nx = v[0] * rw, ny = v[1] * rw;
+        sxMin = fmin(sxMin, nx); sxMax = fmax(sxMax, nx); syMin = fmin(syMin, ny); syMax = fmax(syMax, ny); wMin = fmin(wMin, v[3]);
+        padF = fmax(padF, 1.01 * (X.resid + 1e-15) * (scale * rw) * (1.0 + fmax(fabs(nx), fabs(ny))));
+    }
+    const double wLow = wMin - delta * X.fw;
+    if (!(wLow > 0.5 * wMin)) return none;
+    const double ax = fmax(fabs(sxMin), fabs(sxMax)), ay = fmax(fabs(syMin), fabs(syMax));
+    if (!(ax < 64.0 && ay < 64.0)) return none;
+    const double rl = 1.0001 * (double)(1.0f / (float)wLow);
+    const double px = delta * (X.fx + ax * X.fw) * rl + padF, py = delta * (X.fy + ay * X.fw) * rl + padF;
+    const double pad = 1e-9 * (X.vpW + X.vpH) + 0.0078125 + 1.3e-7 * (1.0 + fmax(ax, ay)) * fmax(X.vpW, X.vpH);
+    const double x0 = (sxMin - px + 1.0) * 0.5 * X.vpW + X.vpX, x1 = (sxMax + px + 1.0) * 0.5 * X.vpW + X.vpX;
+    const double y0 = (1.0 - (syMax + py)) * 0.5 * X.vpH + X.vpY, y1 = (1.0 - (syMin - py)) * 0.5 * X.vpH + X.vpY;
+    const double q[4] = {floor((x0 - pad) * SCR_UNITS) + SCR_BIAS, ceil((x1 + pad) * SCR_UNITS) + SCR_BIAS, floor((y0 - pad) * SCR_UNITS) + SCR_BIAS,
+                         ceil((y1 + pad) * SCR_UNITS) + SCR_BIAS};
+    unsigned f[4];
+    for (int i = 0; i < 4; i++) {
+        if (!(q[i] == q[i])) return none;
+        f[i] = (unsigned)(q[i] < 0.0 ? 0.0 : (q[i] > (double)SCR_MAX ? (double)SCR_MAX : q[i]));
+    }
+    return ScrEntry{f[0] | (f[1] << 16), f[2] | (f[3] << 16)};
+}
+
+XRT_HD ScrEntry screen_packet_rect(int x, int y, int side, int off) {
+    const unsigned x0 = (unsigned)(SCR_UNITS * x - off + SCR_BIAS), x1 = (unsigned)(SCR_UNITS * (x + side - 1) + off + SCR_BIAS);
+    const unsigned y0 = (unsigned)(SCR_UNITS * y - off + SCR_BIAS), y1 = (unsigned)(SCR_UNITS * (y + side - 1) + off + SCR_BIAS);
+    return ScrEntry{x0 | (x1 << 16), y0 | (y1 << 16)};
+}
+XRT_HD bool screen_overlap(unsigned ex, unsigned ey, unsigned rx, unsigned ry) {
+    const bool hit = ((ex & 0xffffu) <= (rx >> 16)) & ((ex >> 16) >= (rx & 0xffffu)) & ((ey & 0xffffu) <= (ry >> 16)) & ((ey >> 16) >= (ry & 0xffffu));
+    return hit | (ex == SCR_NO_CULL);
+}
+
+}
diff --git a/xna-ray-trace_amd/csrc/screen_rects.hip b/xna-ray-trace_amd/csrc/screen_rects.hip
--- /dev/null
+++ b/xna-ray-trace_amd/csrc/screen_rects.hip
@@ -0,0 +1,34 @@
+#include "device_util.h"
+#include "kernels.h"
+#include "screen_rects.h"
+
+namespace xrt {
+
+__global__ __launch_bounds__(64) void k_screen_xf(RayGenParams g, const ObjRec *__restrict__ objects, ScreenXf *__restrict__ out) {
+    if (blockIdx.x == 0 && threadIdx.x == 0) make_screen_xf(g, objects[0].invWorld, *out);
+}
+
+__global__ __launch_bounds__(256) void k_screen_rects(const ScreenXf *__restrict__ xf, const float *__restrict__ refT, int nRefs, uint2 *__restrict__ table) {
+    __shared__ ScreenXf X;
+    static_assert(sizeof(ScreenXf) % 8 == 0 && sizeof(ScreenXf) / 8 <= 256, "one 8-byte word per thread");
+    if (threadIdx.x < sizeof(ScreenXf) / 8) reinterpret_cast<unsigned long long *>(&X)[threadIdx.x] = reinterpret_cast<const unsigned long long *>(xf)[threadIdx.x];
+    __syncthreads();
+    for (size_t r = (size_t)blockIdx.x * blockDim.x + threadIdx.x; r < (size_t)nRefs; r += (size_t)gridDim.x * blockDim.x) {
+        const float *q = refT + r * TRI_REC_WORDS;
+        const float v1[3] = {q[4], q[5], q[6]}, e1[3] = {q[7], q[8], q[9]}, e2[3] = {q[10], q[11], q[12]};
+        const ScrEntry e = screen_entry(X, v1, e1, e2);
+        table[r] = make_uint2(e.x, e.y);
+    }
+}
+
+void launch_screen_rects(const RayGenParams &g, const ObjRec *objects, const float *refT, int nRefs, uint2 *table, hipStream_t st) {
+    static_assert(sizeof(ScreenXf) <= SCREEN_XF_SLOTS * sizeof(uint2), "the frame's part fits behind the table");
+    if (nRefs <= 0) return;
+    ScreenXf *const xf = reinterpret_cast<ScreenXf *>(table + nRefs);
+    int blocks = (nRefs + 255) / 256;
+    if (blocks > 8192) blocks = 8192;
+    hipLaunchKernelGGL(k_screen_xf, dim3(1), dim3(64), 0, st, g, objects, xf);
+    hipLaunchKernelGGL(k_screen_rects, dim3(blocks), dim3(256), 0, st, xf, refT, nRefs, table);
+}
+
+}
diff --git a/xna-ray-trace_amd/csrc/settings.h b/xna-ray-trace_amd/csrc/settings.h
--- a/xna-ray-trace_amd/csrc/settings.h
+++ b/xna-ray-trace_amd/csrc/settings.h
@@ -33,6 +33,7 @@
     int packetGrabMax = 2;
     int packetStaticDiv = 4;
     bool packetQuads = true;
+    bool packetScreen = true;
     bool levelMap = true;
     int nodeCull = 1;
     bool noSingle = false;
@@ -109,6 +110,7 @@
     env_int("XRT_PK_GRAB", c.packetGrabMax, 1, 64);
     env_int("XRT_PK_STATIC", c.packetStaticDiv, 0, 64);
     env_flag("XRT_PK_QUADS", c.packetQuads);
+    env_flag("XRT_PK_SCREEN", c.packetScreen);
     env_flag("XRT_LEVEL_MAP", c.levelMap);
     env_int("XRT_NODE_CULL", c.nodeCull, 0, 2);
     c.noSingle = env_set("XRT_NO_SINGLE");
diff --git a/xna-ray-trace_amd/csrc/xrt_api.cpp b/xna-ray-trace_amd/csrc/xrt_api.cpp
--- a/xna-ray-trace_amd/csrc/xrt_api.cpp
+++ b/xna-ray-trace_amd/csrc/xrt_api.cpp
@@ -24,6 +24,7 @@
 #include "trace_plan.h"
 #include "surface.h"
 #include "compose.h"
+#include "screen_rects.h"
 
 namespace {
 
@@ -446,6 +447,12 @@
         const long long walk = p.skipTiles ? ((long long)lvl_kept_tiles(g) << g.lvl.shift) : (long long)p.P;
         p.pkEntries = (size_t)((walk + 63) / 64);
     }
+    if (p.pkEntries && !batch && s.sceneMode == MODE_SINGLE && s.cfg.packetScreen && g.width <= SCR_MAX_EXTENT && g.height <= SCR_MAX_EXTENT &&
+        s.host->arrays.refN.size() < ((size_t)1 << 30)) {
+        bool ok = true;
+        if (!s.posesOnDevice && !s.host->arrays.objects.empty()) { ScreenXf X; make_screen_xf(g, s.host->arrays.objects[0].invWorld, X); ok = X.ok != 0; }
+        if (ok) p.scrRefs = s.host->arrays.refN.size();
+    }
     const bool laneClosest = (p.pkMask & 5) != 5;
     p.wantFeedback = p.fast && !heap && !adaptive && s.deepMeshes && !s.cfg.noFeedback && laneClosest;
     p.listLong = s.heavyPath > 0.0f || p.wantFeedback;
@@ -527,6 +534,7 @@
             HIPCHECK(hipStreamSynchronize(s->stream));
         }
     }
+    if (P.scrRefs && ((rc = W.scrTable.ensure(P.scrRefs + SCREEN_XF_SLOTS)) || (rc = W.pkRect.ensure(P.pkEntries)))) return rc;
     if (P.useStamps) {
         if ((rc = W.stamps.ensure((size_t)MAX_STAMP_ROWS * STAMP_STRIDE))) return rc;
         if ((rc = F.stampHost.ensure((size_t)MAX_STAMP_ROWS * 2 * sizeof(unsigned long long), hipHostMallocMapped))) return rc;
@@ -569,6 +577,7 @@
     int *overflowFlag;
     bool startEvent;
     unsigned pathEpoch = 0;
+    bool screenDone = false;
 
     static constexpr int QW = 1 + 2 * PACKET_QUEUE_WORDS;
 
@@ -622,6 +631,7 @@
     const int k = T.k, word = shadow ? 1 : 0, R = P.R, nL = P.nL;
     int rc;
     PacketArgs PA = packet_args(s, I, I2, quads);
+    if (quads && quads->table && quads->rect) { PA.scrTable = W.scrTable.p; PA.pkRect = quads->rect; }
     PA.queue += PACKET_QUEUE_WORDS * word;
     if (tileCostDev) {
         PA.tileCost = tileCostDev; PA.tileBase = (int)T.pathBase; PA.tileShift = 9 + (T.gp.samples == 16 ? 4 : (T.gp.samples == 4 ? 2 : 0));
@@ -694,6 +704,7 @@
         W.quadWord ^= 1;
         quads.table = reinterpret_cast<uint2 *>(W.quadTable.p + QUAD_HEAD_WORDS); quads.cap = (int)P.pkEntries;
         quads.count = W.quadTable.p + 64 * W.quadWord; quads.clear = W.quadTable.p + 64 * (W.quadWord ^ 1);
+        if (P.scrRefs && !P.batch) quads.rect = W.pkRect.p;
     }
     if (P.givenHits) {
         Range r("xrt ingest hits");
@@ -710,6 +721,7 @@
         startEvent = false;
     } else
     { Range r("xrt raygen"); launch_raygen(gb, S, rays[0], W.lvlB.p, W.index0.p, cnt, Pc, pathBase, heavy_for(0, hcnt), st, startEvent ? e0 : nullptr, (int)rayCap, &endArgs, &quads); startEvent = false; }
+    if (quads.rect && !screenDone) { Range r("xrt screen rects"); launch_screen_rects(gb, S.objects, S.refT, (int)P.scrRefs, W.scrTable.p, st); screenDone = true; }
     xrt_hit *hitsOf[2] = {W.hits.p, W.hits.p};
     int *flagsOf[2] = {W.hitFlags0.p, W.hitFlags0.p};
     SlotRec *slotOf[2] = {W.slot0.p, W.slot1.p};
@@ -2038,7 +2050,7 @@
             msIntersect += ms; msLongest = std::max(msLongest, (double)ms); launches++;
         }
         if (table && b.size() == 2) {
-            F0.plan.pkEntries = tableCap;
+            F0.plan.pkEntries = tableCap; F0.plan.scrRefs = 0;
             s->quadCtx = 0; s->quadLive = (unsigned long long)hc[0];
         }
     }
@@ -3061,6 +3073,39 @@
     });
 }
 
+int xrt_debug_screen_table(xrt_scene *scene, int32_t host_eval, uint64_t *count, uint32_t *entries_out, int64_t entries_cap) {
+    return guarded("xrt_debug_screen_table", [&]() -> int {
+        int rc = need_device(scene, "xrt_debug_screen_table");
+        if (rc != XRT_OK) return rc;
+        if (!count || entries_cap < 0 || (!entries_out && entries_cap > 0)) return fail(XRT_E_INVALID_ARG, "xrt_debug_screen_table: null argument or negative capacity");
+        BusyGuard guard(scene);
+        if (!guard.owned || scene->frames[0].pending || scene->frames[1].pending) return fail(XRT_E_BUSY, "Current render operation not finished.");
+        *count = 0;
+        if (scene->quadCtx < 0) return XRT_OK;
+        const xrt_scene::WorkBufs &W = scene->frames[scene->quadCtx].w;
+        const FramePlan &P = scene->frames[scene->quadCtx].plan;
+        if (!P.scrRefs || P.batch || !W.scrTable.p) return XRT_OK;
+        HIPCHECK(hipSetDevice(scene->device));
+        HIPCHECK(hipDeviceSynchronize());
+        *count = P.scrRefs;
+        const size_t ne = std::min<size_t>(P.scrRefs, (size_t)entries_cap);
+        if (host_eval) {
+            if (scene->posesOnDevice || scene->host->arrays.objects.empty()) return fail(XRT_E_UNSUPPORTED, "xrt_debug_screen_table: the host does not hold the body's pose");
+            ScreenXf X;
+            make_screen_xf(P.g, scene->host->arrays.objects[0].invWorld, X);
+            const float *refT = scene->host->arrays.refT.data();
+            for (size_t r = 0; r < ne; r++) {
+                const float *q = refT + r * TRI_REC_WORDS;
+                const ScrEntry e = screen_entry(X, q + 4, q + 7, q + 10);
+                entries_out[2 * r] = e.x; entries_out[2 * r + 1] = e.y;
+            }
+            return XRT_OK;
+        }
+        if (ne) HIPCHECK(hipMemcpy(entries_out, W.scrTable.p, ne * 2 * sizeof(uint32_t), hipMemcpyDeviceToHost));
+        return XRT_OK;
+    });
+}
+
 int xrt_split_stats(xrt_scene *scene, uint64_t out[4], int32_t reset) {
     return guarded("xrt_split_stats", [&]() -> int {
         int rc = need_device(scene, "xrt_split_stats");
```

New measurement: 19350, median of 6. +2.7%, better.
